# wuwuz/Pacmann

Measured on AMD Instinct MI355X. Metric: private queries/sec + PIR-scan HBM GB/s, SIFT1M d=128 at 1/2/4/8 GPUs, higher is better.
Workload: dtype u64

## Files before the change

pacmann_amd/csrc/pm_ctx.cpp:

```cpp
#include "pm_host.h"

static thread_local std::string g_err;
namespace pmh {
int fail(int code, const std::string& msg) { g_err = msg; return code; }
}

extern "C" const char* pm_last_error(void) { return g_err.c_str(); }

static constexpr AesTables kAes{};
extern "C" int pm_expand_key(const uint8_t key[16], uint32_t rk[44]) {
  uint8_t w[176];
  memcpy(w, key, 16);
  uint8_t rcon = 1;
  for (int i = 16; i < 176; i += 4) {
    uint8_t t[4] = {w[i - 4], w[i - 3], w[i - 2], w[i - 1]};
    if (i % 16 == 0) {
      uint8_t u = t[0];
      t[0] = kAes.sbox[t[1]] ^ rcon; t[1] = kAes.sbox[t[2]]; t[2] = kAes.sbox[t[3]]; t[3] = kAes.sbox[u];
      rcon = AesTables::gmul(rcon, 2);
    }
    for (int k = 0; k < 4; ++k) w[i + k] = w[i - 16 + k] ^ t[k];
  }
  memcpy(rk, w, 176);
  return 0;
// ... 25 lines not shown
  if (const char* rc = getenv("PM_ROWS_CHECK")) c->rows_check = atoi(rc);
  c->hash_mult.resize(pmk::step_max_e());
  for (size_t w = 0; w < c->hash_mult.size(); ++w) c->hash_mult[w] = row_hash_mult(w);
  if (const char* pw = getenv("PM_PUBLISH_WAIT")) c->publish_wait = pw[0] != '0';
  if (c->publish_wait) {
    for (auto& e : c->done_ring)
      if (hipEventCreateWithFlags(&e, hipEventDisableTiming | hipEventReleaseToSystem) != hipSuccess) {
        delete c;
        return fail(PM_EHIP, "hipEventCreateWithFlags(step completion) failed");
      }
    c->done_ev = c->done_ring[0];
  }
  if (const char* rs = getenv("PM_REPL_SIDE")) c->repl_side = rs[0] != '0';
  const char* ng = getenv("PM_NO_GUESS");
  c->no_guess = ng && ng[0] == '1';
  hipError_t e = hipStreamCreateWithFlags(&c->stream, hipStreamNonBlocking);
  if (e != hipSuccess) { delete c; return fail(PM_EHIP, hipGetErrorString(e)); }
  *out = c;
  return 0;
}
extern "C" void pm_ctx_destroy(pm_ctx* c) { if (c) { (void)hipSetDevice(c->device); delete c; } }
extern "C" int pm_ctx_sync(pm_ctx* c) { HIPCHK(hipStreamSynchronize(c->stream)); HIPCHK(hipGetLastError()); return 0; }
extern "C" int pm_ctx_mem_info(pm_ctx* c, uint64_t* free_b, uint64_t* total_b) {
  if (!c) return fail(PM_EINVAL, "ctx is NULL");
  HIPCHK(hipSetDevice(c->device));
  size_t f = 0, t = 0;
  HIPCHK(hipMemGetInfo(&f, &t));
  if (free_b) *free_b = f;
  if (total_b) *total_b = t;
  return 0;
}
static std::mutex g_tl_mu;
static hipEvent_t g_tl_base = nullptr;
extern "C" int pm_timing_enable(pm_ctx* c, int on) {
  c->timing = on;
  if (on >= 2) {
    std::lock_guard<std::mutex> lk(g_tl_mu);
    if (!g_tl_base) {
      HIPCHK(hipEventCreate(&g_tl_base));
      HIPCHK(hipEventRecord(g_tl_base, c->stream));
    }
  }
  return 0;
}
extern "C" int pm_timing_timeline(pm_ctx* c, const char* path) {
  if (!c || !path) return fail(PM_EINVAL, "NULL argument");
  HIPCHK(hipStreamSynchronize(c->stream));
  std::lock_guard<std::mutex> lk(g_tl_mu);
  if (!g_tl_base) return fail(PM_EINVAL, "no timeline (kernel timing level 2 never enabled)");
  FILE* f = fopen(path, "a");
  if (!f) return fail(PM_EINVAL, std::string("cannot open ") + path);
  for (auto& t : c->launches) {
    float a = 0, b = 0;
    if (hipEventElapsedTime(&a, g_tl_base, t.a) != hipSuccess || hipEventElapsedTime(&b, g_tl_base, t.b) != hipSuccess)
      continue;
    fprintf(f, "%s,%.3f,%.3f,%p\n", t.name.c_str(), a * 1e3, b * 1e3, (void*)c);
  }
  fclose(f);
  return 0;
}
namespace pmh {
std::atomic<int> g_verify_records{0};
std::atomic<int> g_device_loop{-1};
std::atomic<int> g_rccl_timeout_s{-1};
std::atomic<int> g_fault_drl_query{-1};
}
extern "C" int pm_set_option(const char* name, int value) {
  if (!name) return fail(PM_EINVAL, "NULL argument");
  if (!strcmp(name, "verify_records")) { g_verify_records.store(value < 0 ? 0 : value); return 0; }
  if (!strcmp(name, "rccl_timeout_s")) { g_rccl_timeout_s.store(value); return 0; }
  if (!strcmp(name, "device_loop")) { g_device_loop.store(value < 0 ? -1 : value); return 0; }
  if (!strcmp(name, "fault_drl_query")) { g_fault_drl_query.store(value); return 0; }
  if (!strcmp(name, "aes_bs")) { pmk::set_aes_bs(value); return 0; }
  if (!strcmp(name, "fold_rot")) {
    if (value < -1 || value > 1) return fail(PM_EINVAL, "fold_rot takes 1, 0 or -1");
    pmk::set_fold_rot(value);
    return 0;
  }
  if (!strcmp(name, "fold_pack")) {
    if (value < -1 || value > 1) return fail(PM_EINVAL, "fold_pack takes 1, 0 or -1");
    pmk::set_fold_pack(value);
    return 0;
  }
  if (pmk::set_option(name, value)) return fail(PM_EINVAL, std::string("unknown option ") + name);
  return 0;
}
extern "C" int pm_step_plan(const pm_step_shape* in, pm_step_forms* out) {
  if (!in || !out) return fail(PM_EINVAL, "NULL argument");
  if (in->kind > (uint32_t)pmk::STEP_DEVICE || in->nsub == 0 || in->np == 0) return fail(PM_EINVAL, "bad step shape");
  pmk::StepShape s{};
  s.np = in->np; s.nsub = in->nsub; s.np_live = in->np_live; s.max_per_part = in->max_per_part;
  s.maxPH = in->maxPH; s.maxSS = in->maxSS; s.E = in->E; s.ph8 = in->ph8 != 0;
  s.of_caller((int)in->kind, true);
  s.unfused = in->no_fuse != 0; s.no_split = in->no_split != 0; s.no_guess = in->no_guess != 0;
  const pmk::StepPlan p = pmk::step_plan(s, pmk::step_opts());
  static_assert(sizeof out->counter / sizeof out->counter[0] == pmk::STAGE_COUNT, "one slot per launch of a plan");
  *out = pm_step_forms{};
  for (int i = 0; i < pmk::STAGE_COUNT; ++i) {
    const pmk::StepLaunch& l = p.at[i];
    if (l.form < 0) continue;
    out->counter[i] = kHostTimerName[pm_ctx::step_counter(i, l.form)];
    out->grid_x[i] = l.gx; out->grid_y[i] = l.gy; out->block[i] = l.block;
  }
  out->nhelp = p.nhelp; out->nsplit = p.nsplit; out->qw = p.qw; out->np_live = p.np_live; out->cblk = p.cblk;
  out->no_guess = p.no_guess; out->qset = p.qset; out->args_valid = s.args_valid;
  return 0;
}
extern "C" int pm_fold_image_map(uint32_t cs, uint32_t ss, uint32_t E, uint32_t dim, int packed, uint64_t x0,
                                 uint64_t n, uint64_t* row, uint32_t* word, uint8_t* is_packed, uint64_t* nitems,
                                 uint32_t* npk_out) {
  if ((n && (!row || !word || !is_packed)) || !nitems || !npk_out) return fail(PM_EINVAL, "NULL argument");
  if ((cs != 512 && cs != 1024) || ss == 0 || ss % 4 || E < 4 || E % 2) return fail(PM_EINVAL, "not a fold image shape");
  const uint32_t npk = packed ? pmk::fold_pack_shape(E, dim) : 0;
  if (packed && (!npk || cs != 512)) return fail(PM_EINVAL, "these entries have no packed fold image");
  *nitems = pmk::fold_image_words(ss, E, cs, npk) / 2;
  *npk_out = npk;
  if (x0 > *nitems || n > *nitems - x0) return fail(PM_EINVAL, "items past the image");
  pmk::fold_image_map(cs, ss, npk, x0, n, row, word, is_packed);
  return 0;
}
extern "C" int pm_timing_reset(pm_ctx* c) {
  HIPCHK(hipStreamSynchronize(c->stream));
  for (auto& t : c->launches) { c->pool.push_back(t.a); c->pool.push_back(t.b); }
  c->launches.clear();
  for (int i = 0; i < HT_COUNT; ++i) { c->host_n[i] = 0; c->host_ms[i] = 0; }
  return 0;
}
extern "C" int pm_timing_get(pm_ctx* c, const char* name, uint64_t* launches, double* total_ms,
                             double* bytes) {
  HIPCHK(hipStreamSynchronize(c->stream));
  uint64_t n = 0; double ms = 0, by = 0;
  if (strncmp(name, "host_", 5) == 0) {
    for (int i = 0; i < HT_COUNT; ++i)
      if (strcmp(name, kHostTimerName[i]) == 0) { n = c->host_n[i]; ms = c->host_ms[i]; }
    if (launches) *launches = n;
    if (total_ms) *total_ms = ms;
    if (bytes) *bytes = 0;
    return 0;
  }
  for (auto& t : c->launches) {
    if (t.name != name) continue;
    float x = 0;
    HIPCHK(hipEventElapsedTime(&x, t.a, t.b));
    ++n; ms += x; by += t.bytes;
  }
  if (launches) *launches = n;
  if (total_ms) *total_ms = ms;
  if (bytes) *bytes = by;
  return 0;
}

#if defined(PM_STEP_STAMPS) || defined(PM_MR_STAMPS) || defined(PM_ANSWER_STAMPS)
namespace pmh {
int dump_stamps(hipStream_t st, const char* path, const void* hdr, size_t hdr_bytes, const DevBuf& buf, uint64_t count) {
  HIPCHK(hipStreamSynchronize(st));
  std::vector<uint64_t> t(count);
  HIPCHK(hipMemcpy(t.data(), buf.p, count * 8, hipMemcpyDeviceToHost));
  static std::mutex mu;
  std::lock_guard<std::mutex> lk(mu);
  if (FILE* f = fopen(path, "ab")) {
    fwrite(hdr, 1, hdr_bytes, f);
    fwrite(t.data(), 8, count, f);
    fclose(f);
  }
  return 0;
}
// ... 95 lines not shown
```

pacmann_amd/csrc/pm_devloop.cpp:

```cpp
#include "pm_engine.h"

static bool device_loop_on() {
  const int o = g_device_loop.load();
  if (o >= 0) return o != 0;
  static const int env = [] { const char* e = getenv("PM_DEVICE_LOOP"); return e ? atoi(e) : 1; }();
  return env != 0;
}
static uint32_t pow2_at_least(uint64_t x) { uint32_t c = 1; while (c < x) c *= 2; return c; }

struct DrlShape { uint32_t n = 0, qn = 0, kcap = 0, cmask = 0; };
static bool drl_plan(pm_graph** gs, uint32_t S, uint64_t q, int k, int step, int parallel, DrlShape* sh) {
  if (!device_loop_on() || S == 0 || step <= 0 || parallel <= 0 || k <= 0 || (uint32_t)parallel > pmk::kDrlMaxParallel)
    return false;
  const pm_graph* g0 = gs[0];
  const Engine& e0 = g0->pir->e;
  const uint64_t m = g0->m, n = (uint64_t)parallel * m, P = e0.P;
  if (m == 0 || m > 64 || n > pmk::kDrlMaxN || n * m > pmk::kDrlMaxNM || P == 0 || P > 64) return false;
  const uint64_t qn = n / P;
  if (qn == 0 || qn > pmk::step_max_sub_per_part() || e0.B == 0) return false;
  const uint64_t kcap = pow2_at_least((uint64_t)parallel + (uint64_t)step * n);
  if (kcap > pmk::kDrlMaxKcap || (uint64_t)k > kcap || pmk::team_round_lds(kcap, n, m) > 64 * 1024) return false;
  uint64_t maxq = ~0ull;
  for (uint32_t i = 0; i < S; ++i) {
    const pm_graph* g = gs[i];
// ... 105 lines not shown
    HIPCHK(hipMemcpy(g0->dgraph->p, g0->graph, g0->n * m * 4, hipMemcpyHostToDevice));
  }
  CHK(T.sess.reserve(S * sizeof(DrlSess)));
  CHK(T.dummy.reserve((uint64_t)S * P * 8));
  CHK(T.batch.reserve((uint64_t)S * n * 4));
  CHK(T.heap.reserve((uint64_t)S * kcap * 8));
  CHK(T.ktab.reserve((uint64_t)S * 2 * kcap * 8));
  CHK(T.knb.reserve((uint64_t)S * kcap * m * 4));
  CHK(T.kdist.reserve((uint64_t)S * kcap * 4));
  CHK(T.kid.reserve((uint64_t)S * kcap * 4));
  CHK(T.ctabp.reserve(S * 8));
  CHK(T.answers.reserve(std::max<uint64_t>(8, (uint64_t)S * q * k * 8)));
  CHK(G.buf.reserve(T.nsub, S * P, (G.maxPH + 63) / 64, pmk::step_match_blocks(G.maxPH), G.E));
  CHK(T.gid.reserve((uint64_t)T.nsub * 8));
  CHK(T.out.reserve(step_out_bytes(T.nsub, G.E)));
  CHK(T.allq.reserve(std::max<uint64_t>(4, (uint64_t)S * q * dim * 4)));
  CHK(T.part_bytes.reserve(P * 8));
  std::vector<DrlSess> hs(S);
  std::vector<uint64_t> dmy((uint64_t)S * P), ctp(S);
  for (uint32_t i = 0; i < S; ++i) {
    pm_graph* g = gs[i];
    Engine* e = &g->pir->e;
    hs[i] = DrlSess{g->rng.s, g->succ, 0, 0, 0, 0};
    for (uint32_t p = 0; p < P; ++p) dmy[(uint64_t)i * P + p] = e->parts[p].dummy_ctr;
    CHK(ensure_dev_cache(e, sh.cmask, st));
    ctp[i] = (uint64_t)(uintptr_t)e->dcache.p;
  }
  std::vector<uint32_t> sbv(S * P + 1);
  for (uint32_t j = 0; j <= S * P; ++j) sbv[j] = j * sh.qn;
  std::vector<double> pb(P);
  for (uint32_t p = 0; p < P; ++p) pb[p] = answer_bytes(e0.parts[p].d, G.E);
  HIPCHK(hipStreamSynchronize(st));
  HIPCHK(hipMemcpy(T.sess.p, hs.data(), S * sizeof(DrlSess), hipMemcpyHostToDevice));
  HIPCHK(hipMemcpy(T.dummy.p, dmy.data(), dmy.size() * 8, hipMemcpyHostToDevice));
  HIPCHK(hipMemcpy(T.ctabp.p, ctp.data(), S * 8, hipMemcpyHostToDevice));
  HIPCHK(hipMemcpy(G.buf.sb_d.p, sbv.data(), sbv.size() * 4, hipMemcpyHostToDevice));
  HIPCHK(hipMemcpy(T.part_bytes.p, pb.data(), P * 8, hipMemcpyHostToDevice));
  if (q) HIPCHK(hipMemcpy(T.allq.p, queries + (uint64_t)s0 * q * dim, (uint64_t)S * q * dim * 4, hipMemcpyHostToDevice));
  if (G.c->timing >= 2) {
    const uint64_t steps = q * (uint64_t)step;
    CHK(T.step_bytes.reserve(std::max<uint64_t>(8, steps * S * 8)));
    CHK(T.step_real.reserve(std::max<uint64_t>(4, steps * S * 4)));
    HIPCHK(hipMemsetAsync(T.step_bytes.p, 0, std::max<uint64_t>(8, steps * S * 8), st));
    HIPCHK(hipMemsetAsync(T.step_real.p, 0, std::max<uint64_t>(4, steps * S * 4), st));
  }
  HIPCHK(hipEventCreateWithFlags(&T.ev_end, hipEventDisableTiming));
  if (getenv("PM_DRL_STAMPS")) {
    CHK(T.stamps.reserve(16 * 8));
    HIPCHK(hipMemset(T.stamps.p, 0, 16 * 8));
  }
  DrlArgs& A = T.A;
  A.S = S; A.P = P; A.qn = sh.qn; A.n = n; A.m = m; A.parallel = (uint32_t)parallel; A.k = (uint32_t)k;
  A.E = G.E; A.dim = dim; A.kcap = kcap; A.cmask = sh.cmask; A.ns = G.ns; A.q = (uint32_t)q;
  A.N = g0->n; A.PS = e0.PS;
  A.vec16 = (G.E % 2 == 0 && dim % 4 == 0 && m % 4 == 0 && ((m / 4) & (m / 4 - 1)) == 0) ? 1u : 0u;
  A.hdr = T.out.as<PmOutHdr>();
  A.rows = (const uint64_t*)(T.out.as<char>() + (uint64_t)T.nsub * sizeof(PmOutHdr));
  A.subs = G.buf.subs_d.as<PmSub>(); A.gid = T.gid.as<uint64_t>();
  A.graph = g0->dgraph->as<uint32_t>();
  A.start_dist = G.start_dist.as<float>(); A.start_ids = G.start_ids.as<uint32_t>();
  A.sess = T.sess.as<DrlSess>(); A.dummy = T.dummy.as<uint64_t>(); A.batch = T.batch.as<uint32_t>();
  A.heap = T.heap.as<uint64_t>(); A.ktab = T.ktab.as<uint64_t>(); A.knb = T.knb.as<uint32_t>();
  A.kdist = T.kdist.as<float>(); A.kid = T.kid.as<uint32_t>(); A.ctab = T.ctabp.as<uint64_t*>();
  A.answers = T.answers.as<int64_t>(); A.part_bytes = T.part_bytes.as<double>();
  A.step_bytes = T.step_bytes.p ? T.step_bytes.as<double>() : nullptr;
  A.step_real = T.step_real.p ? T.step_real.as<uint32_t>() : nullptr;
  A.stamps = T.stamps.p ? T.stamps.as<uint64_t>() : nullptr;
  T.need.assign(S, 0);
  T.mt.assign(S, 0.0);
  return 0;
}

static int drl_step(DrlTeam& T, const DrlShape& sh) {
  StepGroup& G = T.G;
  pm_ctx* c = G.c;
  const Engine* e0 = G.es[0];
  c->sample_now = c->sample_ctr++ % 7 == 0;
  PmStep S{};
  S.parts = G.parts_d.as<PmPart>();
  G.buf.fill(S, (G.maxPH + 63) / 64, pmk::step_match_blocks(G.maxPH));
  S.subs_h = S.subs;
  S.sb_h = S.sb;
  S.done = G.done.as<uint32_t>();
  S.db = e0->db->as<uint64_t>();
  S.q = nullptr;
  step_out(S, T.out.p, T.nsub);
  S.E = G.E; S.dim = G.dim; S.nsub = T.nsub; S.np = T.S * G.Pl;
  S.np_live = S.np;
  S.token = next_token(G.token);
  step_read_window(S, e0->pf_off, e0->pf_len, G.E);
  S.rows_partial = 1;
  const size_t before = c->launches.size();
  double ans_bytes = 0;
  for (uint32_t li = 0; li < G.Pl; ++li) ans_bytes += answer_bytes(e0->parts[G.lp[li]].d, G.E) * sh.qn * T.S;
  CHK(group_step_launch(G, S, pmk::STEP_DEVICE, sh.qn, T.nsub, ans_bytes));
  for (size_t i = before; i < c->launches.size(); ++i)
    if (c->launches[i].name == "answer" || c->launches[i].name == "match_resolve" || c->launches[i].name == "hint_match")
      T.tl.emplace_back(i, T.seq - 1);
  c->host_add(HT_DEV_STEPS, 0.0);
  return 0;
}

static void drl_round(DrlTeam& T, uint32_t mode, uint64_t qi) {
  pm_ctx* c = T.G.c;
  DrlArgs A = T.A;
  A.mode = mode;
  A.qi = (uint32_t)qi;
  A.seq = T.seq;
  if (mode != DRL_END) T.seq++;
  c->timed_ext("team_round", 0, [&](pmk::PmEvents ev) { pmk::team_round(c->stream, A, ev); }, 2);
}

static int drl_begin(DrlTeam& T, uint64_t qi, uint64_t q) {
  StepGroup& G = T.G;
  hipStream_t st = G.c->stream;
  const uint32_t dim = G.dim;
  HIPCHK(hipMemcpy2DAsync(G.qbuf.p, (size_t)dim * 4, T.allq.as<float>() + qi * dim, (size_t)q * dim * 4,
                          (size_t)dim * 4, T.S, hipMemcpyDeviceToDevice, st));
  const uint64_t nrows = (uint64_t)T.S * G.ns;
  if (nrows)
    G.c->timed("l2_rows", (double)nrows * G.dim * 4, [&] {
      pmk::l2_rows(st, T.gs[0]->dvec->as<float>(), G.dim, nrows, G.start_ids.as<uint32_t>(), G.qbuf.as<float>(), G.dim,
                   G.start_dist.as<float>(), G.ns);
    });
  drl_round(T, DRL_BEGIN, qi);
  return 0;
}
static int drl_query_all(std::vector<std::unique_ptr<DrlTeam>>& teams, const DrlShape& sh, uint64_t qi, uint64_t q,
                         int step) {
  for (auto& t : teams) CHK(drl_begin(*t, qi, q));
  for (int r = 0; r < step; ++r)
    for (auto& t : teams) {
      CHK(drl_step(*t, sh));
      drl_round(*t, r + 1 == step ? DRL_END : DRL_MID, qi);
    }
  HIPCHK(hipGetLastError());
  for (auto& t : teams) {
    for (uint32_t i = 0; i < t->S; ++i) {
      pm_graph* g = t->gs[i];
      Engine* e = &g->pir->e;
      e->FBN += (uint64_t)step * (sh.n / e->B);
      e->QMIP += (uint64_t)step * sh.qn;
      g->total += (uint64_t)step * sh.n;
    }
    t->G.c->host_add(HT_DEV_QUERIES, (double)t->S);
  }
  return 0;
}

static int drl_team_finish(DrlTeam& T, uint64_t q, int k, int64_t* answers) {
  StepGroup& G = T.G;
  HIPCHK(hipStreamSynchronize(G.c->stream));
  const uint32_t S = T.S, P = (uint32_t)G.es[0]->P;
  if (q) HIPCHK(hipMemcpy(answers + (uint64_t)T.s0 * q * k, T.answers.p, (uint64_t)S * q * k * 8, hipMemcpyDeviceToHost));
  std::vector<DrlSess> hs(S);
  std::vector<uint64_t> dmy((uint64_t)S * P);
  HIPCHK(hipMemcpy(hs.data(), T.sess.p, S * sizeof(DrlSess), hipMemcpyDeviceToHost));
  HIPCHK(hipMemcpy(dmy.data(), T.dummy.p, dmy.size() * 8, hipMemcpyDeviceToHost));
  std::vector<uint32_t> fq(P);
  for (uint32_t i = 0; i < S; ++i) {
    pm_graph* g = T.gs[i];
    Engine* e = &g->pir->e;
    g->rng.s = hs[i].rng;
    g->succ = hs[i].succ;
    HIPCHK(hipMemcpy(fq.data(), e->fqn.p, P * 4, hipMemcpyDeviceToHost));
    for (uint32_t p = 0; p < P; ++p) {
      e->parts[p].dummy_ctr = dmy[(uint64_t)i * P + p];
// ... 150 lines not shown
```

pacmann_amd/csrc/pm_engine.cpp:

```cpp
#include "pm_engine.h"

static void derive_key(uint64_t seed, uint64_t part, uint64_t epoch, uint8_t key[16]) {
  uint64_t r1 = hash4(seed, DOM_KEY, part, epoch, 0), r2 = hash4(seed, DOM_KEY, part, epoch, 1);
  memcpy(key, &r1, 8);
  memcpy(key + 8, &r2, 8);
}

static void part_params(PartHost& ph, uint64_t N, uint64_t F) {
  uint64_t target = (uint64_t)(2 * std::sqrt((double)N));
  uint64_t cs = 1;
  while (cs < target) cs *= 2;
  uint64_t ss = (uint64_t)std::ceil((double)N / (double)cs);
  ss = (ss + 3) / 4 * 4;
  const uint64_t thr = 8;
  uint64_t maxq = (uint64_t)(std::sqrt((double)N) * std::log((double)N));
  uint64_t k = (uint64_t)std::ceil(std::log(2.0) * (double)(F + 1));
  uint64_t phn = (k * cs + thr - 1) / thr * thr;
  uint64_t qpc = 3 * (uint64_t)((double)maxq / (double)ss);
  qpc = (qpc + thr - 1) / thr * thr;
  ph.d.N = N;
  ph.d.CS = (uint32_t)cs;
  uint32_t lg = 0; while ((1ull << lg) < cs) ++lg;
  ph.d.log2CS = lg;
  ph.d.SS = (uint32_t)ss;
// ... 23 lines not shown
                         const uint64_t* rawDB, uint64_t F, uint64_t seed, bool batch,
                         uint32_t shard, uint32_t nshards, const Engine* server,
                         const DbGen* gen, uint32_t coord_words) {
  if (nshards == 0 || shard >= nshards) return fail(PM_EINVAL, "shard must be < nshards");
  if (!ctx) return fail(PM_EINVAL, "ctx is NULL");
  if (!rawDB && N && !server && !gen) return fail(PM_EINVAL, "rawDB is NULL");
  if (gen && gen->kind == 1 && (uint64_t)(gen->dim + gen->m) * 4 != Ebytes)
    return fail(PM_EINVAL, "graph entry size must be 4 * (dim + m)");
  if (server && server->ctx->device != ctx->device) return fail(PM_EINVAL, "a client shares the server DB of its own device only");
  if (N == 0) return fail(PM_EINVAL, "DBSize must be > 0");
  if (Ebytes < 8) return fail(PM_EINVAL, "DBEntryByteNum must be >= 8");
  HIPCHK(hipSetDevice(ctx->device));
  g->ctx = ctx; g->is_batch = batch;
  g->N = N; g->Ebytes = Ebytes; g->E = Ebytes / 8; g->F = F; g->seed = seed;
  if (batch) {
    g->B = B;
    g->P = B / 2;
    if (g->P == 0) return fail(PM_EINVAL, "BatchSize must be >= 2");
    g->PS = (N + g->P - 1) / g->P;
    if (g->PS > 1 && g->PS < (1ull << 32)) g->ps_magic = ~0ull / g->PS + 1;
  } else {
    g->P = 1; g->PS = N;
  }
  g->parts.resize(g->P);
  if (g->E > pmk::step_max_e()) return fail(PM_EINVAL, "DBEntrySize above the step kernel's LDS limit");
  g->shard = shard; g->nshards = nshards;
  uint64_t off_tag = 0, off_pp = 0, off_par = 0, off_ridx = 0, off_rval = 0, off_hist = 0, off_ar = 0,
           off_tab = 0, off_tabT = 0, off_cur = 0, off_db = 0;
  for (uint64_t i = 0; i < g->P; ++i) {
    PartHost& ph = g->parts[i];
    uint64_t start = i * g->PS, end = std::min((i + 1) * g->PS, N);
    if (end <= start) return fail(PM_EINVAL, "empty partition (DBSize too small for BatchSize)");
    part_params(ph, end - start, F);
    ph.owned = i % nshards == shard;
    if (!ph.owned) {
      ph.d.seed = seed; ph.d.idx = i;
      continue;
    }
    g->owned_list.push_back((uint32_t)i);
    if (ph.d.CS > 32768) return fail(PM_EINVAL, "ChunkSize > 32768 unsupported (16-bit prep offsets)");
    if (ph.d.SS > pmk::step_max_ss()) return fail(PM_EINVAL, "SetSize above the step kernel's LDS limit");
    if ((uint64_t)ph.d.H >= (1ull << 29)) return fail(PM_EINVAL, "tag space >= 2^29 (util.go:161)");
    ph.d.row0 = off_db; off_db += end - start;
    ph.d.seed = seed; ph.d.idx = i;
    g->maxH = std::max(g->maxH, ph.d.H);
    g->maxCS = std::max(g->maxCS, ph.d.CS);
    g->minCS = std::min(g->minCS, ph.d.CS);
    g->maxPH = std::max(g->maxPH, ph.d.PH);
    g->ph8 = g->ph8 && ph.d.PH % 8 == 0;
    g->maxSS = std::max(g->maxSS, ph.d.SS);
    g->maxRepl = std::max(g->maxRepl, ph.d.SS * ph.d.Qpc);
    ph.d.tag = (uint32_t*)(uintptr_t)off_tag; off_tag += ph.d.H;
    ph.d.pp = (uint32_t*)(uintptr_t)off_pp; off_pp += ph.d.PH;
    ph.d.parity = (uint64_t*)(uintptr_t)off_par; off_par += (uint64_t)ph.d.H * g->E;
    ph.d.ridx = (uint32_t*)(uintptr_t)off_ridx; off_ridx += (uint64_t)ph.d.SS * ph.d.Qpc;
    ph.d.rval = (uint64_t*)(uintptr_t)off_rval; off_rval += (uint64_t)ph.d.SS * ph.d.Qpc * g->E;
    ph.d.hist = (uint32_t*)(uintptr_t)off_hist; off_hist += ph.d.SS;
    ph.d.arena = (uint64_t*)(uintptr_t)off_ar; off_ar += (uint64_t)ph.d.MaxQ * g->E;
    ph.d.tab = (uint16_t*)(uintptr_t)off_tab; off_tab += (uint64_t)ph.d.H * ph.d.SS;
    ph.d.curk = cur_k(ph.d.PH, ph.d.SS);
    ph.d.cur = (uint16_t*)(uintptr_t)off_cur; off_cur += cur_words(ph.d.PH, ph.d.SS, ph.d.curk);
    ph.d.tabT = (uint16_t*)(uintptr_t)off_tabT; off_tabT += tabT_words(ph.d.H, ph.d.SS);
    ph.cache.reserve(ph.d.MaxQ);
  }
  CHK(g->zero16.reserve(64));
  HIPCHK(hipMemset(g->zero16.p, 0, 64));
  if (server) g->db = server->db;
  else CHK(g->db->reserve(std::max<uint64_t>(8, off_db * g->E * 8)));
  for (uint32_t i : server ? std::vector<uint32_t>{} : g->owned_list) {
    const uint64_t start = (uint64_t)i * g->PS, rows = g->parts[i].d.N;
    uint64_t* dst = g->db->as<uint64_t>() + g->parts[i].d.row0 * g->E;
    if (gen && gen->kind == 0)
      pmk::db_synth(ctx->stream, dst, start, rows, (uint32_t)g->E, gen->seed);
    else if (gen)
      pmk::graph_synth(ctx->stream, dst, start, rows, N, gen->dim, gen->m, gen->seed);
    else
      HIPCHK(hipMemcpy(dst, rawDB + start * g->E, rows * g->E * 8, hipMemcpyHostToDevice));
  }
  if (gen) {
    HIPCHK(hipGetLastError());
    HIPCHK(hipStreamSynchronize(ctx->stream));
  }
  uint64_t off_img = 0;
  if (!g->owned_list.empty() && pmk::fold_image_ok(g->minCS, g->maxCS, (uint32_t)g->E)) {
    if (server) {
      g->img_npk = server->img_npk;
    } else if (const uint32_t npk = pmk::fold_pack_slices(g->minCS, g->maxCS, (uint32_t)g->E, coord_words)) {
      DevBuf flag;
      CHK(flag.reserve(64));
      if (pmk::coord_low_zero(ctx->stream, g->db->as<uint64_t>(), off_db, (uint32_t)g->E, coord_words, flag.as<uint32_t>()))
        g->img_npk = npk;
      HIPCHK(hipGetLastError());
    }
    for (uint32_t i : g->owned_list) {
      PmPart& d = g->parts[i].d;
      d.img = (const uint64_t*)(uintptr_t)off_img;
      off_img += pmk::fold_image_words(d.SS, (uint32_t)g->E, (uint32_t)g->maxCS, g->img_npk);
    }
    size_t free_b = 0, total_b = 0;
    if (!server && hipMemGetInfo(&free_b, &total_b) == hipSuccess && off_img * 8 > free_b / 4) {
      for (uint32_t i : g->owned_list) g->parts[i].d.img = nullptr;
      off_img = 0;
    } else if (server && !server->img->p) {
      for (uint32_t i : g->owned_list) g->parts[i].d.img = nullptr;
      off_img = 0;
    }
    if (!off_img) g->img_npk = 0;
  }
  if (off_img) {
    if (server) {
      g->img = server->img;
    } else {
      CHK(g->img->reserve(off_img * 8));
      for (uint32_t i : g->owned_list) {
        const PmPart& d = g->parts[i].d;
        pmk::fold_image(ctx->stream, g->img->as<uint64_t>() + (uintptr_t)d.img, g->db->as<uint64_t>() + d.row0 * g->E,
                        d.N, d.SS, (uint32_t)g->E, (uint32_t)g->maxCS, g->img_npk);
      }
      HIPCHK(hipGetLastError());
      HIPCHK(hipStreamSynchronize(ctx->stream));
    }
  }
  CHK(g->tag.reserve(off_tag * 4));
  CHK(g->pp.reserve(off_pp * 4));
  CHK(g->parity.reserve(off_par * 8));
  CHK(g->ridx.reserve(off_ridx * 4));
  CHK(g->rval.reserve(off_rval * 8));
  CHK(g->hist.reserve(off_hist * 4));
  CHK(g->fqn.reserve(g->P * 4));
  CHK(g->arena.reserve(std::max<uint64_t>(8, off_ar * 8)));
  const bool need_tab = pmk::fold_needs_tab(g->minCS, g->maxCS, (uint32_t)g->E, off_img != 0);
  if (need_tab) CHK(g->tab.reserve(off_tab * 2));
  CHK(g->tabT.reserve(off_tabT * 2));
  CHK(g->cur.reserve(std::max<uint64_t>(2, off_cur * 2)));
  CHK(g->done.reserve(4 * (3 + 16 * 4096)));
  {
    const uint32_t init[3] = {1u << 31, 0, 0};
    HIPCHK(hipMemcpy(g->done.p, init, sizeof init, hipMemcpyHostToDevice));
  }
  {
    g->gran_words = (g->maxPH + 63) / 64;
    const size_t n = (size_t)kArgSubs * (8 + 64 + 2 * g->gran_words + 8) * 8;
    CHK(g->gran.reserve(n));
    HIPCHK(hipMemset(g->gran.p, 0, n));
    CHK(g->err_h.reserve(64));
    memset(g->err_h.p, 0, 64);
  }
  CHK(g->parts_d.reserve(g->P * sizeof(PmPart)));
  CHK(g->owned_d.reserve(std::max<size_t>(1, g->owned_list.size()) * sizeof(PmPart)));
  CHK(g->parts_stage.reserve((g->P + g->owned_list.size()) * sizeof(PmPart)));
  for (uint64_t i = 0; i < g->P; ++i) {
    PmPart& d = g->parts[i].d;
    if (!g->parts[i].owned) continue;
    d.tag = g->tag.as<uint32_t>() + (uintptr_t)d.tag;
    d.pp = g->pp.as<uint32_t>() + (uintptr_t)d.pp;
    d.parity = g->parity.as<uint64_t>() + (uintptr_t)d.parity;
    d.ridx = g->ridx.as<uint32_t>() + (uintptr_t)d.ridx;
    d.rval = g->rval.as<uint64_t>() + (uintptr_t)d.rval;
    d.hist = g->hist.as<uint32_t>() + (uintptr_t)d.hist;
    d.fqn = g->fqn.as<uint32_t>() + i;
    d.arena = g->arena.as<uint64_t>() + (uintptr_t)d.arena;
    d.tabT = g->tabT.as<uint16_t>() + (uintptr_t)d.tabT;
    d.tab = need_tab ? g->tab.as<uint16_t>() + (uintptr_t)d.tab : nullptr;
    d.cur = g->cur.as<uint16_t>() + (uintptr_t)d.cur;
    d.img = off_img ? g->img->as<uint64_t>() + (uintptr_t)d.img : nullptr;
  }
  HIPCHK(hipMemsetAsync(g->fqn.p, 0, g->P * 4, ctx->stream));
  HIPCHK(hipMemsetAsync(g->hist.p, 0, off_hist * 4, ctx->stream));
  HIPCHK(hipStreamSynchronize(ctx->stream));
  return 0;
}
}

static int upload_parts(Engine* g) {
  std::vector<PmPart> v(g->P), w;
  for (uint64_t i = 0; i < g->P; ++i) v[i] = g->parts[i].d;
  for (uint32_t i : g->owned_list) w.push_back(g->parts[i].d);
  HIPCHK(hipMemcpyAsync(g->parts_d.p, v.data(), g->P * sizeof(PmPart), hipMemcpyHostToDevice,
                        g->ctx->stream));
  if (!w.empty())
    HIPCHK(hipMemcpyAsync(g->owned_d.p, w.data(), w.size() * sizeof(PmPart), hipMemcpyHostToDevice,
                          g->ctx->stream));
  HIPCHK(hipStreamSynchronize(g->ctx->stream));
  return 0;
}

static int upload_parts_async(Engine* g, hipStream_t st) {
  if (g->ctx->stream != st && hipStreamQuery(g->ctx->stream) != hipSuccess) {
    if (!g->order_ev) HIPCHK(hipEventCreateWithFlags(&g->order_ev, hipEventDisableTiming));
    HIPCHK(hipEventRecord(g->order_ev, g->ctx->stream));
    HIPCHK(hipStreamWaitEvent(st, g->order_ev, 0));
  }
  const size_t no = g->owned_list.size();
  if (g->stage_ev) HIPCHK(hipEventSynchronize(g->stage_ev));
  else HIPCHK(hipEventCreateWithFlags(&g->stage_ev, hipEventDisableTiming));
  CHK(g->parts_stage.reserve((g->P + no) * sizeof(PmPart)));
  PmPart* h = g->parts_stage.as<PmPart>();
  for (uint64_t i = 0; i < g->P; ++i) h[i] = g->parts[i].d;
  for (size_t i = 0; i < no; ++i) h[g->P + i] = g->parts[g->owned_list[i]].d;
  HIPCHK(hipMemcpyAsync(g->parts_d.p, h, g->P * sizeof(PmPart), hipMemcpyHostToDevice, st));
  if (no) HIPCHK(hipMemcpyAsync(g->owned_d.p, h + g->P, no * sizeof(PmPart), hipMemcpyHostToDevice, st));
  HIPCHK(hipEventRecord(g->stage_ev, st));
  return 0;
// ... 291 lines not shown
                  (unsigned long)row[0], (unsigned long)(it == ph.shadow.end() ? 0 : it->second[0]), (unsigned long)dev[0]);
        }
      }
    }
  }
  for (uint32_t s = 0; s < nsub; ++s) {
    const PmOutHdr& h = g->hdr[s];
    if (h.status == ST_OK) {
      PartHost& ph = g->parts[g->subs[s].part];
      ph.fqn++;
      ph.cache.put(g->subs[s].idx, h.ref);
    } else if (h.status == ST_DUP) {
      const uint32_t r = h.ref - base;
      memcpy(g->rows + (uint64_t)s * E, g->rows + (uint64_t)r * E, E * 8);
      g->hdr[s].dist = g->hdr[r].dist;
    }
  }
#ifdef PM_STAMPS
  {
    std::vector<uint64_t> t(64);
    (void)hipMemcpy(t.data(), g->buf.stamps.p, 64 * 8, hipMemcpyDeviceToHost);
    g->stamp_sum.resize(64, 0.0);
    for (int i = 1; i < 64; ++i)
    {
      const uint64_t base = i >= 48 ? t[48] : i >= 41 ? t[41] : t[0];
      if (t[i] && base && i != 41 && i != 48) g->stamp_sum[i] += (double)(t[i] - base);
    }
    g->stamp_n++;
  }
#endif
}

#if defined(PM_STEP_STAMPS) || defined(PM_MR_STAMPS) || defined(PM_ANSWER_STAMPS)
struct LaunchStamps {
  const char* file = nullptr;
  uint64_t words = 0;
  int begin(const char* f, std::atomic<int>* first, hipStream_t st, StepBufs& B, PmStep& S, uint64_t n) {
    if (!f || (first && first->fetch_add(1) >= 40)) return 0;
    CHK(B.stamps.reserve(n * 8));
    HIPCHK(hipMemsetAsync(B.stamps.p, 0, n * 8, st));
    S.stamps = B.stamps.as<uint64_t>();
    file = f; words = n;
    return 0;
  }
  int end(hipStream_t st, const StepBufs& B, PmStep& S, const void* hdr, size_t hdr_bytes) {
    if (!file) return 0;
    S.stamps = nullptr;
    return dump_stamps(st, file, hdr, hdr_bytes, B.stamps, words);
  }
};
#endif

int step_chain(pm_ctx* c, StepBufs& B, PmStep& S, const pmk::StepShape& shape, uint32_t nreal, double ans_bytes,
               const std::function<int()>& after_resolve) {
  hipStream_t st = c->stream;
  if (shape.desc_shared != (S.subs == S.subs_h && S.sb == S.sb_h))
    return fail(PM_EINVAL, "step_chain: the descriptor is not where the step's shape says");
  const pmk::StepPlan plan = pmk::step_plan(shape, pmk::step_opts());
  S.args_valid = shape.args_valid ? 1u : 0u;
  S.nsplit = plan.nsplit; S.qw = plan.qw; S.np_live = plan.np_live; S.cblk = plan.cblk; S.nhelp = plan.nhelp; S.no_guess = plan.no_guess;
  const uint32_t nsub = S.nsub;
  if (plan.qset) {
    CHK(B.qset.reserve((uint64_t)nsub * plan.qw * 2));
    S.qset = B.qset.as<uint16_t>();
  }
  if (plan.nsplit > 1) {
    CHK(B.part_x.reserve((uint64_t)nsub * plan.nsplit * (S.E & ~3u) * 8));
    S.part_x = B.part_x.as<uint64_t>();
  }
  const bool fused = plan.at[pmk::STAGE_FUSED].form >= 0;
  if (fused) {
    if (plan.nhelp && !B.helpg.p) {
      const size_t nh = (size_t)kArgSubs * kStepHelpMax * kHelpGran * 8;
      CHK(B.helpg.reserve(nh));
      HIPCHK(hipMemsetAsync(B.helpg.p, 0, nh, st));
    }
    S.helpg = B.helpg.as<uint64_t>();
  }
  auto run = [&](int stage, const char* name, double bytes) {
    const int form = plan.at[stage].form;
    if (form < 0) return;
    c->timed_ext(name, bytes, [&](pmk::PmEvents ev) { pmk::step_launch(st, S, plan, stage, ev); }, 2);
    c->host_add(pm_ctx::step_counter(stage, form), stage == pmk::STAGE_FUSED ? plan.nhelp : 0.0);
  };
#ifdef PM_STEP_STAMPS
  LaunchStamps ss;
  const uint32_t sh[4] = {plan.at[pmk::STAGE_FUSED].gx, nsub, pmk::step_match_blocks(shape.maxPH), S.np};
  if (fused) CHK(ss.begin(getenv("PM_STAMP_FILE"), nullptr, st, B, S, (uint64_t)sh[0] * 8));
#endif
  run(pmk::STAGE_FUSED, "step", ans_bytes);
#ifdef PM_STEP_STAMPS
  CHK(ss.end(st, B, S, sh, sizeof sh));
#endif
#ifdef PM_MR_STAMPS
  LaunchStamps ms;
  static std::atomic<int> mr_steps{0};
  const uint64_t mh = S.np;
  if (plan.at[pmk::STAGE_MR].form >= 0) CHK(ms.begin(getenv("PM_MR_STAMPS"), &mr_steps, st, B, S, mh * 8));
#endif
  run(pmk::STAGE_MR, "match_resolve", (double)nreal * shape.maxPH);
#ifdef PM_MR_STAMPS
  CHK(ms.end(st, B, S, &mh, sizeof mh));
#endif
  run(pmk::STAGE_MATCH, "hint_match", (double)nreal * shape.maxPH);
  run(pmk::STAGE_RESOLVE, "resolve", 0);
  if (after_resolve) CHK(after_resolve());
  run(pmk::STAGE_GATHER, "gather", ans_bytes);
#ifdef PM_ANSWER_STAMPS
  LaunchStamps as;
  static std::atomic<int> ans_steps{0};
  const uint64_t ah = nsub;
  if (!fused) CHK(as.begin(getenv("PM_ANSWER_STAMPS"), &ans_steps, st, B, S, ah * 8));
#endif
  run(pmk::STAGE_ANSWER, "answer", plan.nsplit > 1 ? 0 : ans_bytes);
#ifdef PM_ANSWER_STAMPS
  CHK(as.end(st, B, S, &ah, sizeof ah));
#endif
  return 0;
}

int engine_step(Engine* g, const float* q_dev, uint32_t dim) {
  auto t_begin = Clock::now();
  pm_ctx* c = g->ctx;
  hipStream_t st = c->stream;
  const uint32_t nsub = (uint32_t)g->subs.size();
  if (nsub == 0) return 0;
  const uint64_t E = g->E;
  const uint32_t words = (g->maxPH + 63) / 64, cblk = pmk::step_match_blocks(g->maxPH);
  StepBufs& B = g->buf;
  CHK(B.reserve(nsub, (uint32_t)g->P, words, cblk, E));
  const size_t dsub = nsub * sizeof(PmSub);
  CHK(B.desc_h.reserve(dsub + (g->P + 1) * 4));
  CHK(B.out_h.reserve(step_out_bytes(nsub, E)));
  char* dh = B.desc_h.as<char>();
  memcpy(dh, g->subs.data(), dsub);
  memcpy(dh + dsub, g->sb.data(), (g->P + 1) * 4);
  PmStep S{};
  S.parts = g->parts_d.as<PmPart>();
  S.subs_h = (const PmSub*)dh;
  S.sb_h = (const uint32_t*)(dh + dsub);
  B.fill(S, words, cblk);
  if (words <= g->gran_words) {
    uint64_t* gb = g->gran.as<uint64_t>();
    S.recg = gb;
    S.specg = gb + kArgSubs * 8;
    S.bitsg = gb + kArgSubs * (8 + 64);
    S.resg = gb + kArgSubs * (8 + 64 + 2 * (uint64_t)g->gran_words);
    S.err_h = g->err_h.as<uint32_t>();
  }
  S.done = g->done.as<uint32_t>();
#ifdef PM_STAMPS
  CHK(B.stamps.reserve(g->P * 64 * 8));
  HIPCHK(hipMemsetAsync(B.stamps.p, 0, g->P * 64 * 8, st));
  S.stamps = B.stamps.as<uint64_t>();
#endif
  S.db = g->db->as<uint64_t>();
  S.q = q_dev;
  step_out(S, B.out_h.p, nsub);
  S.E = (uint32_t)E; S.dim = q_dev ? dim : 0; S.nsub = nsub; S.np = (uint32_t)g->P;
  S.token = next_token(g->step_token);
  step_read_window(S, g->pf_off, g->pf_len, E);
  S.rows_partial = host_rows_partial(c, g->rows_partial);
  uint32_t nreal = 0;
  for (auto& x : g->subs) nreal += x.kind == SUB_REAL;
  pmk::StepShape shape{};
  shape.np = (uint32_t)g->P; shape.nsub = nsub; shape.maxPH = g->maxPH; shape.maxSS = g->maxSS; shape.E = (uint32_t)E; shape.ph8 = g->ph8;
  for (uint64_t p = 0; p < g->P; ++p) {
    const uint32_t n = g->sb[p + 1] - g->sb[p];
    shape.max_per_part = std::max(shape.max_per_part, n);
    shape.np_live += n > 0;
  }
  shape.of_caller(pmk::STEP_ENGINE, S.recg && S.err_h);
  shape.unfused = c->no_fuse || c->debug_sync; shape.no_split = c->no_split; shape.no_guess = c->no_guess;
  if (shape.args_valid) {
    memcpy(S.subs_a, g->subs.data(), dsub);
    memcpy(S.sb_a, g->sb.data(), (g->P + 1) * 4);
  }
  double ans_bytes = 0;
  for (auto& x : g->subs)
    if (x.kind == SUB_REAL || x.kind == SUB_DUMMY) ans_bytes += answer_bytes(g->parts[x.part].d, E);
  std::function<int()> dump_res;
  if (c->debug_sync) dump_res = [&]() -> int {
    std::vector<PmRes> rr(nsub);
    HIPCHK(hipMemcpy(rr.data(), S.res, nsub * sizeof(PmRes), hipMemcpyDeviceToHost));
    for (uint32_t s = 0; s < nsub; ++s) {
      const PmPart& d = g->parts[g->subs[s].part].d;
      const PmRes& r = rr[s];
      const bool bad = (r.status == ST_OK && (r.hit >= d.PH || r.slot >= d.MaxQ || r.chunk >= d.SS || r.ing >= d.Qpc)) ||
                       (r.status == ST_CACHED && r.slot >= d.MaxQ) || (r.status == ST_DUP && r.slot >= nsub) ||
                       (r.status > ST_SKIP) || (r.status > ST_ERANGE && r.status < ST_DUMMY);
      fprintf(stderr, "[pm] res s=%u part=%u kind=%u idx=%lu -> st=%u hit=%u chunk=%u ing=%u tag=%u pp=%u slot=%u flags=%u%s\n",
              s, g->subs[s].part, g->subs[s].kind, (unsigned long)g->subs[s].idx, r.status, r.hit, r.chunk, r.ing,
              r.tag, r.pp, r.slot, r.flags, bad ? "  <-- BAD" : "");
    }
    return 0;
  };
  CHK(step_chain(c, B, S, shape, nreal, ans_bytes, dump_res));
  g->step_seq = c->record_done(st);
  HIPCHK(hipGetLastError());
  c->host_add(HT_STEP_LAUNCH, ms_since(t_begin));
  CHK(wait_and_post(g, S, nsub, t_begin));
  if (S.err_h && *(volatile uint32_t*)S.err_h) {
    *(volatile uint32_t*)S.err_h = 0;
    return fail(PM_EHIP, "k_step: a hand-off wait timed out (results of this step are invalid)");
  }
  return 0;
}
}

static void add_sub(Engine* g, uint32_t p, bool real, uint64_t local, uint64_t gid) {
  PartHost& ph = g->parts[p];
  if (!ph.owned) return;
  PmSub s{p, SUB_NONE, 0};
  if (!real) {
    s.kind = SUB_DUMMY; s.idx = ph.dummy_ctr++;
  } else {
    s.kind = SUB_REAL; s.idx = local;
    if (const uint32_t* slot = ph.cache.find(local)) { s.kind = SUB_HOSTCACHE; s.idx = *slot; }
  }
  g->subs.push_back(s);
  g->sub_gid.push_back(gid);
}
static void begin_step(Engine* g) {
  g->subs.clear(); g->sub_gid.clear();
  g->sb.assign(g->P + 1, 0);
}
static void close_partition(Engine* g, uint32_t p) {
  for (uint64_t i = p + 1; i <= g->P; ++i) g->sb[i] = (uint32_t)g->subs.size();
}

namespace pmh {
void print_stamps(const Engine& e) {
#ifdef PM_STAMPS
  if (!e.stamp_n) return;
  fprintf(stderr, "[pm-stamps] mean shader clocks since kernel start over %lu steps (1-40 k_resolve part 0, 42-47 k_match, 49-63 k_answer):", (unsigned long)e.stamp_n);
  for (size_t i = 1; i < e.stamp_sum.size(); ++i)
    if (e.stamp_sum[i] > 0) fprintf(stderr, " %zu:%.0f", i, e.stamp_sum[i] / e.stamp_n);
  fprintf(stderr, "\n");
#else
// ... 411 lines not shown
```

pacmann_amd/csrc/pm_engine.h:

```cpp
#pragma once
#include "pm_host.h"

#include <functional>

struct DbGen;
struct Engine;
struct pm_graph;
struct StepGroup;
struct StepBufs;
struct ShardComb;

namespace pmh {
int engine_create(pm_ctx* ctx, Engine* g, uint64_t N, uint64_t Ebytes, uint64_t B,
                  const uint64_t* rawDB, uint64_t F, uint64_t seed, bool batch,
                  uint32_t shard = 0, uint32_t nshards = 1, const Engine* server = nullptr,
                  const DbGen* gen = nullptr, uint32_t coord_words = 0);
int ensure_host_cache(Engine* g);
int engine_prep_host(Engine* g, uint64_t p0, uint64_t p1, std::vector<uint64_t>& todo,
                     hipStream_t st = nullptr);
int engine_prep_launch(pm_ctx* c, const Engine* g, const PmPart* dp, int np, const PmPart* host_parts,
                       uint32_t clients = 1, bool sync = true);
int wait_done(pm_ctx* sc, uint64_t seq);
int poll_done(pm_ctx* sc, uint64_t seq, bool* ready);
int wait_step(pm_ctx* c, const PmOutHdr* hdr, uint32_t nsub, uint32_t token, const char* rows,
// ... 74 lines not shown
  bool emplace(uint64_t k, uint32_t v) {
    if (find(k)) return false;
    put(k, v);
    return true;
  }
  template <class F> void for_each(F&& f) const {
    for (const Slot& x : slot) if (x.gen == cur) f(x.key, x.val);
  }
};

struct StepBufs {
  DevBuf subs_d, sb_d, bits, cand, meta, spec, res_d, ans, part_x, stamps;
  DevBuf qset;
  DevBuf helpg;
  HostBuf desc_h, out_h;
  int reserve(uint32_t nsub, uint32_t np, uint32_t words, uint32_t cblk, uint64_t E) {
    CHK(subs_d.reserve(nsub * sizeof(PmSub)));
    CHK(sb_d.reserve((np + 1) * 4));
    CHK(bits.reserve((uint64_t)nsub * words * 8));
    CHK(cand.reserve((uint64_t)nsub * cblk * 6 * 4));
    CHK(meta.reserve((uint64_t)nsub * 2 * 4));
    CHK(spec.reserve((uint64_t)nsub * 64 * 4));
    CHK(res_d.reserve(nsub * sizeof(PmRes)));
    CHK(ans.reserve((uint64_t)nsub * E * 8));
    return 0;
  }
  void fill(PmStep& S, uint32_t words, uint32_t cblk) const {
    S.subs = subs_d.as<PmSub>();
    S.sb = sb_d.as<uint32_t>();
    S.bits = bits.as<uint64_t>();
    S.cand = cand.as<uint32_t>();
    S.meta = meta.as<uint32_t>();
    S.spec = spec.as<uint32_t>();
    S.res = res_d.as<PmRes>();
    S.ans = ans.as<uint64_t>();
    S.words = words;
    S.cblk = cblk;
  }
};
static inline size_t step_out_bytes(uint32_t nsub, uint64_t E) { return nsub * sizeof(PmOutHdr) + (size_t)nsub * E * 8; }
static inline void step_out(PmStep& S, void* out, uint32_t nsub) {
  S.hdr_h = (PmOutHdr*)out;
  S.rows_h = (uint64_t*)((char*)out + nsub * sizeof(PmOutHdr));
}
static inline uint32_t next_token(uint32_t& token) {
  if (++token == 0) ++token;
  return token;
}
static inline void step_read_window(PmStep& S, size_t pf_off, size_t pf_len, uint64_t E) {
  const size_t off = std::min<size_t>(pf_off, E * 8);
  const size_t end = std::min<size_t>(E * 8, off + std::min<size_t>(pf_len, E * 8));
  S.pf_w0 = (uint32_t)(off / 8);
  S.pf_w1 = (uint32_t)((end + 7) / 8);
}
static inline uint32_t host_rows_partial(const pm_ctx* c, bool partial) {
  return partial && !c->verify_rows && !c->debug_cache ? 1u : 0u;
}
struct PartHost {
  PmPart d{};
  bool owned = true;
  uint64_t epoch_ctr = 0, fqn = 0, dummy_ctr = 0;
  uint64_t maxq64 = 0;
  FlatMap cache;
  std::unordered_map<uint64_t, std::vector<uint64_t>> shadow;
};

struct Engine {
  pm_ctx* ctx = nullptr;
  bool is_batch = false;
  uint64_t N = 0, E = 0, Ebytes = 0, F = 0, seed = 0;
  uint64_t B = 0, P = 1, PS = 0;
  uint64_t ps_magic = 0;
  uint64_t part_of(uint64_t id) const {
    return ps_magic && id < (1ull << 32) ? (uint64_t)(((unsigned __int128)id * ps_magic) >> 64) : id / PS;
  }
  uint32_t shard = 0, nshards = 1;
  bool skipPrep = false;
  uint64_t FBN = 0, QMIP = 0, Support = 0, prepCount = 0;
  double prepTime = 0, storage = 0, commOn = 0, commOff = 0;

  std::shared_ptr<DevBuf> db = std::make_shared<DevBuf>();
  std::shared_ptr<DevBuf> img = std::make_shared<DevBuf>();
  uint32_t img_npk = 0;
  DevBuf zero16, parts_d, owned_d, tag, pp, parity, ridx, rval, hist, fqn, arena, tab, tabT, cur, done, gran;
  HostBuf parts_stage;
  hipEvent_t stage_ev = nullptr;
  hipEvent_t order_ev = nullptr;
  uint32_t gran_words = 0;
  std::vector<uint32_t> owned_list;
  DevBuf qoffs, ans_srv;
  StepBufs buf;
  std::vector<double> stamp_sum;
  uint64_t stamp_n = 0;
  uint32_t step_token = 0;
  uint64_t step_seq = 0;
  size_t pf_off = 0, pf_len = ~size_t(0);
  bool rows_partial = false;
  HostBuf err_h, src_h;
  HostBuf stage_h;
  hipEvent_t dev_ev = nullptr;
  ~Engine() {
    if (dev_ev) (void)hipEventDestroy(dev_ev);
    if (stage_ev) (void)hipEventDestroy(stage_ev);
    if (order_ev) (void)hipEventDestroy(order_ev);
  }
  std::vector<PartHost> parts;
  uint32_t maxH = 0, maxPH = 0, maxSS = 0, maxRepl = 0, maxCS = 0, minCS = ~0u;
  bool ph8 = true;

  std::vector<PmSub> subs;
  std::vector<uint32_t> sb;
  std::vector<uint64_t> sub_gid;
  PmOutHdr* hdr = nullptr;
  uint64_t* rows = nullptr;
  std::vector<std::vector<uint64_t>> pq;
  FlatMap resp_map;
  std::vector<uint64_t> resp_rows;
  std::vector<float> resp_dist;
  std::vector<uint8_t> resp_ok;
  std::vector<char> slow;
  uint64_t qn = 0;
  uint64_t prep_gen = 0;
  std::vector<uint64_t> zero_row;
  DevBuf dcache;
  uint32_t dcache_cmask = 0;
  bool cache_on_dev = false, dcache_valid = false;
};

static inline double answer_bytes(const PmPart& d, uint64_t E) {
  const double rows = std::min((double)d.SS, (double)d.N / (double)d.CS);
  return rows * (double)E * 8 + 4.0 * d.SS + 8.0 * E;
}

struct DbGen { int kind; uint64_t seed; uint32_t dim, m; };

struct pm_batchpir { Engine e; ~pm_batchpir() { print_stamps(e); } };

struct SplitMix {
  uint64_t s;
  uint64_t next() { s += 0x9e3779b97f4a7c15ULL; uint64_t z = s;
    z = (z ^ (z >> 30)) * 0xbf58476d1ce4e5b9ULL; z = (z ^ (z >> 27)) * 0x94d049bb133111ebULL;
    return z ^ (z >> 31); }
  uint64_t intn(uint64_t n) { return next() % n; }
};
struct VD { float dist; int64_t id; };

struct pm_graph {
  pm_ctx* ctx = nullptr;
  uint64_t n = 0, dim = 0, m = 0;
  bool nonprivate = false, skipPrep = false;
  uint64_t pir_seed = 0;
  SplitMix rng{0};
  std::shared_ptr<const std::vector<float>> vec_own;
  std::shared_ptr<const std::vector<uint32_t>> graph_own;
  const float* vectors = nullptr;
  const uint32_t* graph = nullptr;
  std::shared_ptr<DevBuf> dvec = std::make_shared<DevBuf>();
  std::shared_ptr<DevBuf> dgraph = std::make_shared<DevBuf>();
  uint32_t shard = 0, nshards = 1;
  bool synth = false;
  uint64_t data_seed = 0;
  DevBuf dstartvec;
  std::vector<uint8_t> okv;
  const uint32_t* true_nb(uint64_t id, uint32_t* tmp) const {
    if (!synth) return graph + id * m;
    const uint64_t kg = sm64(data_seed + DOM_SYNTH_NB);
// ... 94 lines not shown
```

pacmann_amd/csrc/pm_group.cpp:

```cpp
#include "pm_engine.h"

struct SpinBarrier {
  std::atomic<uint32_t> count{0}, gen{0};
  uint32_t n = 1;
  void wait() {
    const uint32_t g0 = gen.load(std::memory_order_acquire);
    if (count.fetch_add(1, std::memory_order_acq_rel) + 1 == n) {
      count.store(0, std::memory_order_relaxed);
      gen.fetch_add(1, std::memory_order_release);
    } else {
      while (gen.load(std::memory_order_acquire) == g0) std::this_thread::yield();
    }
  }
};

struct ShardComb {
  pm_combine_fn fn = nullptr;
  void* user = nullptr;
  bool model_peers = false;
  uint32_t NG = 1;
  uint64_t* const* bufs = nullptr;
  std::atomic<uint64_t> ticket{0};
  std::atomic<bool> abort{false};
};
// ... 100 lines not shown
    if (!ss.ok || ss.step != G.nstep) staged = false;
    nsub += ss.n;
  }
  if (staged && pmk::step_args_fit(nsub, np)) staged = false;
  G.nstep++;
  PmSub* const stage = G.stage_h.as<PmSub>();
  if (staged) {
    uint32_t off = 0;
    for (uint32_t s = 0; s < G.S; ++s) {
      const StepGroup::SessStage& ss = G.stg[s];
      G.base[s] = off;
      const uint32_t n = in[s] ? ss.n : 0;
      if (n && off != s * G.stride) memmove(stage + off, stage + (uint64_t)s * G.stride, (size_t)n * sizeof(PmSub));
      for (uint32_t li = 0; li < G.Pl; ++li) G.sb.push_back(G.sb.back() + (in[s] ? ss.pc[li] : 0));
      if (in[s]) {
        max_per_part = std::max(max_per_part, ss.maxpp);
        np_live += ss.live;
        ans_bytes += ss.bytes;
        nreal += ss.nreal;
      }
      off += n;
    }
  } else {
    G.subs.clear();
    for (uint32_t s = 0; s < G.S; ++s) {
      Engine* e = G.es[s];
      G.base[s] = (uint32_t)G.subs.size();
      for (uint32_t li = 0; li < G.Pl; ++li) {
        const uint32_t p = G.lp[li];
        if (in[s]) {
          for (uint32_t j = e->sb[p]; j < e->sb[p + 1]; ++j) {
            PmSub x = e->subs[j];
            x.part = s * G.Pl + li;
            G.subs.push_back(x);
            if (x.kind == SUB_REAL || x.kind == SUB_DUMMY) ans_bytes += answer_bytes(e->parts[p].d, G.E);
            nreal += x.kind == SUB_REAL;
          }
          const uint32_t n = e->sb[p + 1] - e->sb[p];
          max_per_part = std::max(max_per_part, n);
          np_live += n > 0;
        }
        G.sb.push_back((uint32_t)G.subs.size());
      }
      need = std::max(need, in[s] ? (uint32_t)G.subs.size() - G.base[s] : 0u);
    }
    nsub = (uint32_t)G.subs.size();
  }
  G.nsub = nsub;
  if (G.stage_on && need > G.stride) {
    G.stride = (need + 7) & ~7u;
    CHK(G.stage_h.reserve((size_t)G.S * G.stride * sizeof(PmSub) + (size_t)(np + 1) * 4));
    if (G.stg.size() != G.S) G.stg.resize(G.S);
  }
  if (nsub == 0) return 0;
  const uint32_t words = (G.maxPH + 63) / 64, cblk = pmk::step_match_blocks(G.maxPH);
  StepBufs& B = G.buf;
  CHK(B.reserve(nsub, np, words, cblk, G.E));
  const size_t dsub = nsub * sizeof(PmSub);
  char* dh;
  if (staged) {
    dh = G.stage_h.as<char>();
    memcpy(dh + dsub, G.sb.data(), (np + 1) * 4);
  } else {
    CHK(B.desc_h.reserve(dsub + (np + 1) * 4));
    dh = B.desc_h.as<char>();
    memcpy(dh, G.subs.data(), dsub);
    memcpy(dh + dsub, G.sb.data(), (np + 1) * 4);
  }
  PmStep S{};
  S.parts = G.parts_d.as<PmPart>();
  S.subs_h = (const PmSub*)dh;
  S.sb_h = (const uint32_t*)(dh + dsub);
  B.fill(S, words, cblk);
  if (!pmk::step_args_fit(nsub, np)) {
    CHK(G.desc_d.reserve(dsub + (np + 1) * 4));
    HIPCHK(hipMemcpyAsync(G.desc_d.p, dh, dsub + (np + 1) * 4, hipMemcpyHostToDevice, st));
    S.subs_h = G.desc_d.as<PmSub>();
    S.sb_h = (const uint32_t*)(G.desc_d.as<char>() + dsub);
    S.subs = const_cast<PmSub*>(S.subs_h);
    S.sb = const_cast<uint32_t*>(S.sb_h);
  }
  S.done = G.done.as<uint32_t>();
  Engine* e0 = G.es[0];
  S.db = e0->db->as<uint64_t>();
  S.q = nullptr;
  if (G.comb) {
    CHK(G.out_d.reserve(step_out_bytes(nsub, G.E)));
    step_out(S, G.out_d.p, nsub);
  } else {
    CHK(B.out_h.reserve(step_out_bytes(nsub, G.E)));
    step_out(S, B.out_h.p, nsub);
  }
  S.E = G.E; S.dim = G.dim; S.nsub = nsub; S.np = np;
  S.np_live = np_live;
  if (pmk::step_args_fit(nsub, np)) {
    memcpy(S.subs_a, G.subs.data(), dsub);
    memcpy(S.sb_a, G.sb.data(), (np + 1) * 4);
  }
  S.token = next_token(G.token);
  step_read_window(S, e0->pf_off, e0->pf_len, G.E);
  S.rows_partial = host_rows_partial(c, G.rows_partial);
  return group_step_launch(G, S, pmk::STEP_SHARED, max_per_part, nreal, ans_bytes);
}

static void prefetch_session(StepGroup& G, uint32_t s, const pm_graph* g) {
  const Engine* e = G.es[s];
  const uint32_t n = (uint32_t)e->subs.size();
  const PmOutHdr* hdr = G.buf.out_h.as<PmOutHdr>() + G.base[s];
  const char* rows = G.buf.out_h.as<char>() + (size_t)G.nsub * sizeof(PmOutHdr) + (size_t)G.base[s] * G.E * 8;
  for (uint32_t j = 0; j < n; j += 2) __builtin_prefetch(hdr + j);
  for (uint32_t j = 0; j < n; ++j)
    for (uint32_t w = G.pf_w0; w < G.pf_w1; w += 8) __builtin_prefetch(rows + ((size_t)j * G.E + w) * 8);
  if (g->graph)
    for (size_t b = 0; b < g->batch.size(); ++b) __builtin_prefetch(&g->graph[(uint64_t)g->batch[b] * g->m]);
}

static int group_collect(StepGroup& G, uint32_t s) {
  Engine* e = G.es[s];
  const uint32_t n = (uint32_t)e->subs.size();
  for (uint32_t j = 0; j < n; ++j)
    if (e->subs[j].kind == SUB_REAL) e->parts[e->subs[j].part].cache.prefetch(e->subs[j].idx);
  PmOutHdr* hdr = G.buf.out_h.as<PmOutHdr>();
  uint64_t* rows = (uint64_t*)(G.buf.out_h.as<char>() + (size_t)G.nsub * sizeof(PmOutHdr));
  auto t_wait = Clock::now();
  CHK(wait_step(e->ctx, hdr + G.base[s], n, G.token, (const char*)(rows + (uint64_t)G.base[s] * G.E),
                (size_t)G.E * 8, (size_t)G.pf_w0 * 8, (size_t)(G.pf_w1 - G.pf_w0) * 8, G.seq, G.c));
  e->ctx->host_add(HT_STEP_WAIT, ms_since(t_wait));
  auto tp = Clock::now();
  post_results(e, hdr, rows, n, G.base[s], G.token);
  e->ctx->host_add(HT_STEP_POST, ms_since(tp));
  return 0;
}

static int group_start_dist(StepGroup& G, pm_graph** gs) {
  hipStream_t st = G.c->stream;
  float* qst = G.qstage.as<float>();
  HIPCHK(hipMemcpyAsync(G.qbuf.p, qst, (uint64_t)G.S * G.dim * 4, hipMemcpyHostToDevice, st));
  const uint64_t nrows = (uint64_t)G.S * G.ns;
  if (nrows) {
    const bool ids = gs[0]->dvec->p != nullptr;
    G.c->timed("l2_rows", (double)nrows * G.dim * 4, [&] {
      pmk::l2_rows(st, ids ? gs[0]->dvec->as<float>() : G.start_vec.as<float>(), G.dim, nrows,
                   ids ? G.start_ids.as<uint32_t>() : nullptr, G.qbuf.as<float>(), G.dim, G.start_dist.as<float>(),
                   G.ns);
    });
    HIPCHK(hipMemcpyAsync(qst + (uint64_t)G.S * G.dim, G.start_dist.p, nrows * 4, hipMemcpyDeviceToHost, st));
  }
  HIPCHK(hipStreamSynchronize(st));
  return 0;
}

namespace pmh {
int prep_clients(pm_ctx* c, DevBuf& pbuf, const std::vector<uint32_t>& lp, const std::vector<Engine*>& who,
                        const std::vector<double*>* mt, HostBuf* stage, hipEvent_t* stage_ev) {
  if (who.empty()) return 0;
  for (Engine* e : who)
    if ((e->img->p != nullptr) != (who[0]->img->p != nullptr))
      return fail(PM_EINVAL, "grouped clients were created with and without the fold image");
  auto t0 = Clock::now();
  std::vector<PmPart> hp;
  std::vector<uint64_t> todo;
  for (Engine* e : who) {
    e->FBN = 0; e->QMIP = 0;
    CHK(engine_prep_host(e, 0, e->P, todo, c->stream));
  }
  for (uint32_t p : lp)
    for (Engine* e : who) hp.push_back(e->parts[p].d);
// ... 898 lines not shown
```

pacmann_amd/csrc/pm_host.h:

```cpp
#define PM_HOST_TU 1
#pragma once
#include "pm_internal.h"
#include "pm_aes.h"
#include "../../include/pacmann.h"

#include <dlfcn.h>
#include <hip/hip_runtime.h>
#include <rccl/rccl.h>

#include <algorithm>
#include <atomic>
#include <cstdio>
#include <cstdlib>
#include <chrono>
#include <condition_variable>
#include <cmath>
#include <cstring>
#include <memory>
#include <string>
#include <mutex>
#include <thread>
#include <unordered_map>
#include <vector>

using namespace pm;

struct DevBuf;

namespace pmh {
int fail(int code, const std::string& msg);
extern std::atomic<int> g_verify_records;
extern std::atomic<int> g_device_loop;
extern std::atomic<int> g_rccl_timeout_s;
extern std::atomic<int> g_fault_drl_query;
int dump_stamps(hipStream_t st, const char* path, const void* hdr, size_t hdr_bytes, const DevBuf& buf, uint64_t count);
}
using namespace pmh;

#define HIPCHK(x)                                                                         \
  do {                                                                                    \
    hipError_t e_ = (x);                                                                  \
    if (e_ != hipSuccess)                                                                 \
      return fail(PM_EHIP, std::string(#x) + ": " + hipGetErrorString(e_));               \
  } while (0)
#define CHK(x)            \
  do {                    \
    int r_ = (x);         \
    if (r_ != 0) return r_; \
  } while (0)

struct DevBuf {
  void* p = nullptr;
  size_t n = 0;
  ~DevBuf() { if (p) (void)hipFree(p); }
  int reserve(size_t bytes) {
    if (bytes <= n) return 0;
    if (p) { (void)hipFree(p); p = nullptr; n = 0; }
    if (bytes == 0) return 0;
    hipError_t e = hipMalloc(&p, bytes);
    if (e != hipSuccess) return fail(PM_ENOMEM, "hipMalloc(" + std::to_string(bytes) + "): " + hipGetErrorString(e));
    n = bytes;
    return 0;
  }
  template <class T> T* as() const { return (T*)p; }
};
struct HostBuf {
  void* p = nullptr;
  size_t n = 0;
  ~HostBuf() { if (p) (void)hipHostFree(p); }
  int reserve(size_t bytes) {
    if (bytes <= n) return 0;
    if (p) { (void)hipHostFree(p); p = nullptr; n = 0; }
    hipError_t e = hipHostMalloc(&p, bytes, hipHostMallocCoherent | hipHostMallocMapped);
    if (e != hipSuccess) return fail(PM_ENOMEM, std::string("hipHostMalloc: ") + hipGetErrorString(e));
    memset(p, 0, bytes);
    n = bytes;
    return 0;
  }
  template <class T> T* as() const { return (T*)p; }
};

enum HostTimer : int { HT_STEP_LAUNCH, HT_STEP_WAIT, HT_STEP_POST, HT_BATCH_QUERY, HT_GVI_PARSE, HT_SEARCH_KNN, HT_KNN_INIT, HT_KNN_BATCH, HT_KNN_UPDATE, HT_KNN_FINAL, HT_WAIT_FIRST, HT_WAIT_ALL, HT_ROWS_SEEN, HT_ROWS_TORN, HT_WAIT_DONE, HT_COMBINE, HT_COMBINE_TURN, HT_PATH_MATCH, HT_PATH_MATCH_PART, HT_PATH_MATCH_PART8, HT_PREP_SETS, HT_REC_VERIFIED, HT_REC_BAD, HT_REC_DROPPED, HT_REC_FAILED, HT_REC_PEER, HT_REC_UNEXPLAINED, HT_FOLD_ROT512, HT_FOLD_ROT1024, HT_FOLD_OTHER, HT_FOLD_PIPE, HT_FOLD_BLK, HT_FOLD_GATHER, HT_FOLD_ROT512P, HT_DEV_STEPS, HT_DEV_QUERIES, HT_KNN_BATCH_FALLBACK, HT_PATH_STEP, HT_PATH_RESOLVE_LDS, HT_PATH_RESOLVE_G, HT_PATH_MR_S2, HT_PATH_MR_S4, HT_PATH_MR_GENERAL, HT_PATH_GATHER, HT_PATH_ANSWER_P5, HT_PATH_ANSWER_P, HT_PATH_ANSWER_S, HT_PATH_ANSWER_G, HT_COUNT };
static const char* const kHostTimerName[HT_COUNT] = {"host_step_launch", "host_step_wait", "host_step_post", "host_batch_query", "host_gvi_parse", "host_search_knn", "host_knn_init", "host_knn_batch", "host_knn_update", "host_knn_final", "host_wait_first_token", "host_wait_all_tokens", "host_rows_seen", "host_rows_torn", "host_wait_done", "host_combine", "host_combine_turn", "host_path_match", "host_path_match_part", "host_path_match_part8", "host_prep_sets", "host_records_verified", "host_records_bad", "host_records_dropped", "host_records_failed", "host_records_peer", "host_records_unexplained", "host_fold_rot512", "host_fold_rot1024", "host_fold_other", "host_fold_pipe", "host_fold_blk", "host_fold_gather", "host_fold_rot512p", "host_dev_steps", "host_dev_queries", "host_knn_batch_fallback", "host_path_step", "host_path_resolve_lds", "host_path_resolve_g", "host_path_mr_s2", "host_path_mr_s4", "host_path_mr_general", "host_path_gather", "host_path_answer_p5", "host_path_answer_p", "host_path_answer_s", "host_path_answer_g"};
static_assert(HT_PATH_ANSWER_G - HT_PATH_STEP + 1 == pmk::FORM_COUNT, "one counter per step form, in the order of pmk::FORM_*");

struct TimedLaunch { std::string name; hipEvent_t a, b; double bytes; };

struct pm_ctx {
  int device = 0;
  hipStream_t stream = nullptr;
  int timing = 0;
  bool sample_now = true;
  uint64_t sample_ctr = 0;
  bool no_fuse = false;
  bool no_split = false;
  bool no_guess = false;
  bool verify_rows = false;
  bool debug_cache = false;
  bool log_steps = false;
  bool debug_sync = false;
  bool repl_side = true;
  hipStream_t side = nullptr;
  hipEvent_t side_ev[2] = {};
  std::mutex side_mu;
  int rows_check = 2;
  std::vector<uint64_t> hash_mult;
  bool publish_wait = true;
  static constexpr uint32_t kDoneRing = 64;
  hipEvent_t done_ev = nullptr;
  hipEvent_t done_ring[kDoneRing] = {};
  std::atomic<uint64_t> done_rec{0}, done_seen{0};
  std::mutex done_mu, rec_mu;
  uint64_t record_done(hipStream_t st) {
    if (!publish_wait) return 0;
    std::lock_guard<std::mutex> lk(rec_mu);
    const uint64_t seq = done_rec.load(std::memory_order_relaxed) + 1;
    (void)hipEventRecord(done_ring[seq % kDoneRing], st);
    done_rec.store(seq, std::memory_order_release);
    return seq;
  }
  std::string last_kernel;
  uint64_t host_n[HT_COUNT] = {};
  double host_ms[HT_COUNT] = {};
  void host_add(HostTimer t, double ms) { host_n[t]++; host_ms[t] += ms; }
  static HostTimer step_counter(int stage, int form) {
    if (stage != pmk::STAGE_MATCH) return (HostTimer)(HT_PATH_STEP + form);
    return form == pmk::MATCH_PART8 ? HT_PATH_MATCH_PART8 : form == pmk::MATCH_PART ? HT_PATH_MATCH_PART : HT_PATH_MATCH;
  }
  std::vector<TimedLaunch> launches;
  std::vector<hipEvent_t> pool;
  hipEvent_t ev() {
    if (!pool.empty()) { hipEvent_t e = pool.back(); pool.pop_back(); return e; }
    hipEvent_t e; (void)hipEventCreate(&e); return e;
  }
  template <class F> void timed(const char* name, double bytes, F&& f, int level = 1) {
    last_kernel = name;
    if (debug_sync) {
      f();
      hipError_t e = hipStreamSynchronize(stream);
      if (e != hipSuccess) fprintf(stderr, "[pm] kernel %s failed: %s\n", name, hipGetErrorString(e));
      return;
    }
    if (timing < level) { f(); return; }
    TimedLaunch t{name, ev(), ev(), bytes};
    (void)hipEventRecord(t.a, stream);
    f();
    (void)hipEventRecord(t.b, stream);
    launches.push_back(t);
  }
  template <class F> void timed_ext(const char* name, double bytes, F&& f, int level) {
    last_kernel = name;
    if (debug_sync) { timed(name, bytes, [&] { f(pmk::PmEvents{}); }, level); return; }
    if (timing < level || (timing == 3 && level == 2 && !sample_now)) { f(pmk::PmEvents{}); return; }
    TimedLaunch t{name, ev(), ev(), bytes};
    f(pmk::PmEvents{t.a, t.b});
    launches.push_back(t);
  }
  ~pm_ctx() {
    for (auto& t : launches) { (void)hipEventDestroy(t.a); (void)hipEventDestroy(t.b); }
    for (auto e : pool) (void)hipEventDestroy(e);
    for (auto e : done_ring) if (e) (void)hipEventDestroy(e);
    for (auto e : side_ev) if (e) (void)hipEventDestroy(e);
    if (side) (void)hipStreamDestroy(side);
    if (stream) (void)hipStreamDestroy(stream);
  }
};
// ... 5 lines not shown
```

pacmann_amd/csrc/pm_internal.h:

```cpp
#pragma once
#include <hip/hip_runtime.h>
#include <stdint.h>

#include <string>

#if defined(__HIP_DEVICE_COMPILE__) && !defined(PM_HOST_TU)
#define PM_G __attribute__((address_space(1)))
#else
#define PM_G
#endif

namespace pm {

constexpr uint32_t kDefaultProgramPoint = 0x7fffffffu;
constexpr uint64_t kDefaultValue = 0xdeadbeefULL;
constexpr uint16_t kSkip = 0xffffu;
constexpr int kBlock = 256;

enum : uint64_t { DOM_KEY = 1, DOM_REPL = 2, DOM_DUMMY = 3, DOM_SYNTH_DB = 9, DOM_SYNTH_VEC = 10, DOM_SYNTH_NB = 11 };
__host__ __device__ inline uint64_t sm64(uint64_t x) {
  uint64_t z = x + 0x9e3779b97f4a7c15ULL;
  z = (z ^ (z >> 30)) * 0xbf58476d1ce4e5b9ULL;
  z = (z ^ (z >> 27)) * 0x94d049bb133111ebULL;
  return z ^ (z >> 31);
// ... 27 lines not shown
  uint64_t seed;
  uint64_t epoch;
  uint64_t idx;
  uint32_t CS, log2CS, SS, PH, Qpc, H, MaxQ, curk;
  uint32_t rk[44];
  PM_G uint32_t* tag;
  PM_G uint32_t* pp;
  PM_G uint64_t* parity;
  PM_G uint32_t* ridx;
  PM_G uint64_t* rval;
  PM_G uint32_t* hist;
  PM_G uint32_t* fqn;
  PM_G uint64_t* arena;
  PM_G uint16_t* tab;
  PM_G uint16_t* tabT;
  PM_G uint16_t* cur;
  const PM_G float* qv;
  const PM_G uint64_t* img;
};

__host__ __device__ inline uint64_t tabT_index(uint32_t H, uint32_t t, uint32_t c) {
  return ((uint64_t)(c >> 3) * H + t) * 8 + (c & 7);
}
struct FoldImageSrc { uint64_t row; uint32_t word; bool packed; };
__host__ __device__ inline uint64_t tabT_words(uint32_t H, uint32_t SS) { return (uint64_t)((SS + 7) / 8) * 8 * H; }

#ifndef PM_CUR_K
#define PM_CUR_K 0
#endif
__host__ __device__ inline uint32_t cur_k(uint32_t PH, uint32_t SS) {
  return PM_CUR_K ? PM_CUR_K : ((uint64_t)PH * 2 > (uint64_t)SS * 128 ? 1u : 2u);
}
__host__ __device__ inline uint32_t cur_blocks(uint32_t PH) { return (PH + 7) >> 3; }
__host__ __device__ inline uint64_t cur_index(uint32_t PH, uint32_t K, uint32_t c, uint32_t h) {
  return K == 2 ? (((uint64_t)(c >> 1) * cur_blocks(PH) + (h >> 3)) * 2 + (c & 1)) * 8 + (h & 7)
                : (((uint64_t)(c / K) * cur_blocks(PH) + (h >> 3)) * K + (c % K)) * 8 + (h & 7);
}
__host__ __device__ inline uint64_t cur_row(uint32_t PH, uint32_t K, uint32_t c) { return cur_index(PH, K, c, 0); }
__host__ __device__ inline uint32_t cur_row_off(uint32_t K, uint32_t h) { return (h >> 3) * 8 * K + (h & 7); }
__host__ __device__ inline uint64_t cur_words(uint32_t PH, uint32_t SS, uint32_t K) {
  return (uint64_t)((SS + K - 1) / K) * cur_blocks(PH) * 8 * K;
}

enum : uint32_t { SUB_NONE = 0, SUB_REAL = 1, SUB_DUMMY = 2, SUB_HOSTCACHE = 3 };
enum : uint32_t {
  ST_OK = 0, ST_EBUDGET = 1, ST_ECHUNK = 2, ST_ENOHIT = 3, ST_ERANGE = 4,
  ST_DUMMY = 8, ST_CACHED = 9, ST_DUP = 10, ST_SKIP = 11
};
struct PmSub {
  uint32_t part, kind;
  uint64_t idx;
};
struct PmRes {
  uint32_t status, hit, chunk, ing;
  uint32_t tag, pp;
  uint32_t slot;
  uint32_t flags;
};
constexpr uint64_t kCsumMix = 0x9E3779B97F4A7C15ull;
__host__ __device__ inline uint64_t row_hash_mult(uint64_t w) { return sm64(w ^ 0x5851F42D4C957F2Dull) | 1ull; }
struct alignas(16) PmOutHdr {
  uint32_t status, ref;
  float dist;
  uint32_t token;
  uint64_t csum, pad;
};
#ifndef PM_KARG_SUBS
#define PM_KARG_SUBS 112
#endif
constexpr uint32_t kArgSubs = PM_KARG_SUBS, kArgParts = PM_KARG_SUBS > 1 ? 32 : 1;
constexpr uint32_t kStepHelpMax = 3, kHelpWords = 256, kHelpGran = 2 * kHelpWords + 8;
struct PmStep {
  const PM_G PmPart* parts;
  const PM_G PmSub* subs_h;
  const PM_G uint32_t* sb_h;
  PM_G PmSub* subs;
  PM_G uint32_t* sb;
  PM_G uint64_t* bits;
  PM_G uint32_t* cand;
  PM_G PmRes* res;
  PM_G uint64_t* ans;
  PM_G uint32_t* done;
  const PM_G uint64_t* db;
  const PM_G float* q;
  PM_G PmOutHdr* hdr_h;
  PM_G uint64_t* rows_h;
  PM_G uint64_t* stamps;
  PM_G uint32_t* meta;
  PM_G uint32_t* spec;
  PM_G uint64_t* recg;
  PM_G uint64_t* specg;
  PM_G uint64_t* bitsg;
  PM_G uint64_t* resg;
  PM_G uint64_t* helpg;
  uint32_t nhelp;
  PM_G uint32_t* err_h;
  uint32_t words, E, dim, nsub, np, cblk;
  uint32_t np_live;
  uint32_t pf_w0, pf_w1;
  uint32_t rows_partial;
  uint32_t no_guess;
  uint32_t nsplit;
  PM_G uint64_t* part_x;
  PM_G uint16_t* qset;
  uint32_t qw;
  uint32_t args_valid;
  uint32_t token;
  uint32_t sb_a[kArgParts + 1];
  PmSub subs_a[kArgSubs];
};

__host__ __device__ inline uint32_t drl_hash(uint32_t k) {
  uint64_t x = k;
  x ^= x >> 33; x *= 0xff51afd7ed558ccdULL; x ^= x >> 33;
  return (uint32_t)x;
}
struct DrlSess {
  uint64_t rng;
  uint64_t succ;
  uint32_t nknown, nheap;
  uint32_t pad0, pad1;
};
enum : uint32_t { DRL_BEGIN = 0, DRL_MID = 1, DRL_END = 2 };
struct DrlArgs {
  uint32_t S, P, qn, n, m, parallel, k, E, dim, kcap, cmask, ns, mode, q, qi, seq;
  uint32_t vec16;
  uint64_t N, PS;
  const PmOutHdr* hdr;
  const uint64_t* rows;
  PmSub* subs;
  uint64_t* gid;
  const uint32_t* graph;
  const float* start_dist;
  const uint32_t* start_ids;
  DrlSess* sess;
  uint64_t* dummy;
  uint32_t* batch;
  uint64_t* heap;
  uint64_t* ktab;
  uint32_t* knb;
  float* kdist;
  uint32_t* kid;
  uint64_t* const* ctab;
  int64_t* answers;
  const double* part_bytes;
  double* step_bytes;
  uint32_t* step_real;
  uint64_t* stamps;
};

struct KnbArgs {
  const float* vec;
  const uint32_t* graph;
  const uint32_t* start;
  const float* queries;
  uint32_t nq, ns, dim, m, k, max_step, parallel, kcap;
  int64_t* ids;
  int64_t* steps;
  uint32_t* needs_host;
};

}

namespace pmk {
using namespace pm;
void prep_init(hipStream_t st, const PmPart* dparts, int nparts, uint32_t maxH, uint32_t maxRepl,
               uint32_t E, bool zero_state);
void prep_offsets(hipStream_t st, const PmPart* dparts, int nparts, uint32_t maxH, uint32_t maxSS);
void set_aes_bs(int v);
enum : int { FOLD_GATHER = 0, FOLD_ROT512 = 1, FOLD_ROT1024 = 2, FOLD_PIPE = 3, FOLD_BLK = 4, FOLD_ROT512P = 5 };
int fold_form(uint32_t minCS, uint32_t maxCS, uint32_t E, bool have_img, uint32_t npk = 0);
void set_fold_rot(int v);
int prep_fold(hipStream_t st, const PmPart* dparts, int nparts, uint32_t maxH, const uint64_t* db,
              uint32_t E, uint32_t minCS, uint32_t maxCS, const uint64_t* zero16, uint32_t clients = 1,
              bool have_img = false, uint32_t minH = 0, uint32_t npk = 0);
void prep_repl(hipStream_t st, const PmPart* dparts, int nparts, uint32_t maxRepl,
               const uint64_t* db, uint32_t E);
bool fold_image_ok(uint32_t minCS, uint32_t maxCS, uint32_t E);
bool fold_needs_tab(uint32_t minCS, uint32_t maxCS, uint32_t E, bool have_img);
uint64_t fold_image_words(uint32_t SS, uint32_t E, uint32_t CS, uint32_t npk = 0);
void fold_image(hipStream_t st, uint64_t* img, const uint64_t* part_rows, uint64_t N, uint32_t SS, uint32_t E,
                uint32_t CS, uint32_t npk = 0);
void set_fold_pack(int v);
uint32_t fold_pack_shape(uint32_t E, uint32_t dim);
uint32_t fold_pack_slices(uint32_t minCS, uint32_t maxCS, uint32_t E, uint32_t dim);
bool coord_low_zero(hipStream_t st, const uint64_t* rows, uint64_t nrows, uint32_t E, uint32_t dim, uint32_t* flag);
void fold_image_map(uint32_t CS, uint32_t SS, uint32_t npk, uint64_t x0, uint64_t n, uint64_t* row, uint32_t* word,
                    uint8_t* packed);
struct PmEvents { hipEvent_t a = nullptr, b = nullptr; };
int set_option(const char* name, int value);
struct StepOpts { int match_part, match_part8, match_resolve, answer_waves, answer_nt, answer_pair, gather_split, step_help; };
StepOpts step_opts();
uint32_t step_match_blocks(uint32_t maxPH);
enum : int { STEP_ENGINE = 0, STEP_SHARED = 1, STEP_DEVICE = 2 };
inline bool step_args_fit(uint32_t nsub, uint32_t np) { return nsub <= kArgSubs && np <= kArgParts; }
struct StepShape {
  uint32_t np, nsub, np_live, max_per_part, maxPH, maxSS, E;
  bool ph8;
  bool args_valid;
  bool desc_shared;
  bool granules;
  bool unfused;
  bool no_split, no_guess;
  void of_caller(int kind, bool have_granules) {
    args_valid = kind != STEP_DEVICE && step_args_fit(nsub, np);
    desc_shared = kind == STEP_DEVICE || (kind == STEP_SHARED && !args_valid);
    granules = kind == STEP_ENGINE && have_granules;
  }
};
enum : int { MATCH_SUB = 0, MATCH_PART = 1, MATCH_PART8 = 2 };
enum : int { FORM_STEP = 0, FORM_RESOLVE_LDS, FORM_RESOLVE_G, FORM_MR_S2, FORM_MR_S4, FORM_MR_GENERAL,
             FORM_GATHER, FORM_ANSWER_P5, FORM_ANSWER_P, FORM_ANSWER_S, FORM_ANSWER_G, FORM_COUNT };
enum : int { STAGE_FUSED = 0, STAGE_MR, STAGE_MATCH, STAGE_RESOLVE, STAGE_GATHER, STAGE_ANSWER, STAGE_COUNT };
struct StepLaunch { int form = -1; uint32_t gx = 0, gy = 1, block = 0; };
struct StepPlan {
  StepLaunch at[STAGE_COUNT];
  uint32_t nhelp, nsplit, qw, np_live, cblk, no_guess;
  bool qset;
};
StepPlan step_plan(const StepShape& s, const StepOpts& O);
void step_launch(hipStream_t st, const PmStep& S, const StepPlan& plan, int stage, PmEvents ev = {});
uint32_t step_max_sub_per_part();
uint32_t step_max_ss();
uint32_t step_max_e();
void server_answer(hipStream_t st, const PmPart* dpart, const uint32_t* offs, uint32_t nq,
                   uint32_t SS, const uint64_t* db, uint32_t E, uint64_t* out);
void l2_rows(hipStream_t st, const float* rows, uint64_t row_stride_floats, uint64_t nrows,
             const uint32_t* row_ids, const float* q, uint32_t dim, float* out, uint64_t seglen = 0);
void ip_rows(hipStream_t st, const uint32_t* rows, uint64_t nrows, const uint32_t* q, uint32_t dim,
             uint32_t* per_row, uint32_t* sum);
void ip_fill(hipStream_t st, uint32_t* rows, uint64_t N, uint32_t D, uint64_t r0 = 0);
void db_synth(hipStream_t st, uint64_t* dst, uint64_t r0, uint64_t rows, uint32_t E, uint64_t db_seed);
void gather_rows(hipStream_t st, const uint64_t* const* src, uint64_t n, uint32_t E, uint64_t* out);
void graph_synth(hipStream_t st, uint64_t* dst, uint64_t r0, uint64_t rows, uint64_t n, uint32_t dim, uint32_t m,
                 uint64_t seed);
void graph_synth_vecs(hipStream_t st, const uint64_t* ids, uint64_t nids, uint32_t dim, uint64_t seed, float* out);
void pack_records(hipStream_t st, const int32_t* map, uint32_t nrec, const PmOutHdr* hdr, const uint64_t* rows,
                  uint32_t E, uint32_t w0, uint32_t W, uint64_t* rec, uint32_t nsub, uint32_t* st2, uint64_t errw);
void synth_records(hipStream_t st, const int32_t* map, const uint64_t* ids, uint32_t nrec, uint32_t npos,
                   const float* qbuf, uint32_t dim, uint32_t m, uint64_t n, uint64_t seed, uint32_t w0, uint32_t W,
                   uint64_t* rec);
void prf_batch(hipStream_t st, const uint32_t* rk, const uint64_t* tags, const uint64_t* xs,
               uint64_t n, uint64_t* out);
void team_round(hipStream_t st, const DrlArgs& A, PmEvents ev = {});
uint32_t team_round_lds(uint32_t kcap, uint32_t n, uint32_t m);
constexpr uint32_t kDrlMaxKcap = 4096, kDrlMaxN = 256, kDrlMaxNM = 8192, kDrlMaxParallel = 8;
constexpr uint32_t kKnbMaxBatch = 256, kKnbMaxM = 64, kKnbMaxLds = 160 * 1024 - 512;
uint32_t knn_batch_kcap(uint64_t parallel, uint64_t max_step, uint64_t m);
uint64_t knn_batch_lds(uint32_t kcap, uint32_t dim, uint32_t nb, uint32_t ns);
bool knn_batch_ok(uint64_t dim, uint64_t m, uint64_t ns, uint64_t max_step, uint64_t parallel);
void knn_batch(hipStream_t st, const KnbArgs& A);
uint32_t knn_pad_dim(uint32_t dim);
uint32_t knn_top();
uint32_t prune_max_list();
uint32_t prune_max_dim();
uint32_t prune_max_m();
void to_bf16(hipStream_t st, const float* rows, uint64_t n, uint32_t dim, uint32_t dp, void* out, float* norms);
void knn_prefilter(hipStream_t st, const void* X, const float* xn, uint64_t N, const void* Q, const float* qn,
                   uint64_t M, uint32_t dp, uint32_t* out, uint32_t* out_hi = nullptr);
void knn_rerank(hipStream_t st, const float* X, uint64_t N, uint32_t dim, const float* Q, uint64_t M,
                const uint32_t* cand, uint32_t K, bool self_base, uint32_t* out, float* dist, uint32_t* len);
void to_bf16x2(hipStream_t st, const float* rows, uint64_t n, uint32_t dim, uint32_t dp, void* hi, void* lo,
               float* norms, uint32_t* maxnorm);
void knn_prefilter_x3(hipStream_t st, const void* Xh, const void* Xl, const float* xn, uint64_t N, const void* Qh,
                      const void* Ql, const float* qn, uint64_t M, uint32_t dp, uint32_t* out, float* tau,
                      uint32_t* out_hi = nullptr);
float knn_cert_rel(uint32_t dp);
void knn_rerank_cert(hipStream_t st, const float* X, uint64_t N, uint32_t dim, const float* Q, uint64_t M,
                     const uint32_t* cand, uint32_t K, bool self_base, uint32_t* out, float* dist, uint32_t* len,
                     const float* qn, const float* tau, const uint32_t* maxnorm, uint32_t dp, uint64_t* list,
                     uint64_t* nlist, float* eps_out = nullptr);
void knn_brute(hipStream_t st, const float* X, uint64_t N, uint32_t dim, const float* Q, const uint64_t* list,
               uint64_t nlist, uint32_t K, bool self_base, uint32_t* out, float* dist, uint32_t* len);
void prune(hipStream_t st, const float* X, uint32_t dim, const uint32_t* verts, uint64_t nverts,
           const uint64_t* offs, uint64_t stride, const uint32_t* lens, const uint32_t* ids, uint32_t m,
           float alpha, uint32_t* out, uint32_t* out_len, uint32_t* err, const uint32_t* sorted_pos = nullptr,
           const float* dist_g = nullptr);
void cand_dist(hipStream_t st, const float* X, uint32_t dim, const uint32_t* verts, uint64_t nverts,
               const uint64_t* offs, const uint32_t* lens, const uint32_t* ids, float* dist_g);
uint32_t knn_pad_dim_wide(uint32_t dim);
void knn_prefilter_x3_w(hipStream_t st, const void* Xh, const void* Xl, const float* xn, uint64_t N, const void* Qh,
                        const void* Ql, const float* qn, uint64_t M, uint32_t dp, uint32_t* out, float* tau,
                        uint32_t* out_hi = nullptr);
void knn_brute_w(hipStream_t st, const float* X, uint64_t N, uint32_t dim, const float* Q, const uint64_t* list,
                 uint64_t nlist, uint32_t K, bool self_base, uint32_t* out, float* dist, uint32_t* len);
void prune_w(hipStream_t st, const float* X, uint32_t dim, const uint32_t* verts, uint64_t nverts,
             const uint64_t* offs, uint64_t stride, const uint32_t* lens, const uint32_t* ids, uint32_t m,
             float alpha, uint32_t* out, uint32_t* out_len, uint32_t* err, const uint32_t* sorted_pos = nullptr,
             const float* dist_g = nullptr);
}
```

pacmann_amd/csrc/pm_kernels.hip:

```cpp
#include <atomic>
#include "pm_aes.h"
#include "pm_aes_bs.h"
#include "pm_internal.h"

namespace pm {
#ifndef PM_PREP_NT
#define PM_PREP_NT 0
#endif


__device__ __forceinline__ uint32_t xor3(uint32_t a, uint32_t b, uint32_t c) {
  return __builtin_amdgcn_bitop3_b32(a, b, c, 0x96);
}
__device__ __forceinline__ uint4 xor4(uint4 a, uint4 b) {
  return make_uint4(a.x ^ b.x, a.y ^ b.y, a.z ^ b.z, a.w ^ b.w);
}

#ifndef PM_OFFS_CHUNKS
#define PM_OFFS_CHUNKS 8
#endif
constexpr int kOffsChunksPerBlock = PM_OFFS_CHUNKS;
constexpr int kOffsBlock = 1024;

#ifndef PM_OFFS_TILES
// ... 524 lines not shown
        uint32_t v[2][8];
#pragma unroll
        for (uint32_t pp = 0; pp < 2; ++pp) {
          const uint32_t ph = p0 + pp;
          uint32_t o;
          if constexpr (NCH == 4) o = __builtin_amdgcn_perm(tv[k].y, tv[k].x, psel[ph]);
          else o = __builtin_amdgcn_perm(0u, tv[k], psel[ph]);
          o = min(o, (uint32_t)CS);
          const uint32_t a = o * (LINE * 4) + cso[ph];
          const uint4 x0 = *reinterpret_cast<const uint4*>(lds0 + a);
          const uint4 x1 = *reinterpret_cast<const uint4*>(lds0 + (a ^ 16u));
          v[pp][0] = x0.x; v[pp][1] = x0.y; v[pp][2] = x0.z; v[pp][3] = x0.w;
          v[pp][4] = x1.x; v[pp][5] = x1.y; v[pp][6] = x1.z; v[pp][7] = x1.w;
        }
#pragma unroll
        for (int t = 0; t < 8; ++t)
          acc[k][t] = xor3(acc[k][t], v[0][t], v[1][t]);
      }
    }
    asm volatile("s_waitcnt vmcnt(0)" ::: "memory");
    __syncthreads();
#pragma unroll
    for (int k = 0; k < HPL; ++k) tv[k] = tn[k];
    skip_idle(tv);
  }
#pragma unroll
  for (int k = 0; k < HPL; ++k) {
    const uint32_t v = vl + k * kFoldThreads;
    if (v >= v1) continue;
    const bool inB = v >= vb;
    PM_G uint64_t* const par = (inB ? PB.parity : PA.parity) + (uint64_t)(v - (inB ? vb : hA)) * E;
    PM_G uint32_t* dst = reinterpret_cast<PM_G uint32_t*>(par + w);
    if (slice < npk) {
      typedef uint32_t u32x4 __attribute__((ext_vector_type(4)));
#pragma unroll
      for (int t = 0; t < 8; t += 2) {
        PM_G u32x4* const d = reinterpret_cast<PM_G u32x4*>(dst + 8 * (j ^ (t >> 2)) + 2 * (t & 3));
        const u32x4 x = {acc[k][t] << 16, acc[k][t] & 0xffff0000u, acc[k][t + 1] << 16, acc[k][t + 1] & 0xffff0000u};
        if (PM_PREP_NT) __builtin_nontemporal_store(x, d);
        else *d = x;
      }
    } else {
#pragma unroll
      for (int t = 0; t < 8; ++t) {
        PM_G uint32_t* const d = dst + 4 * (j ^ (t >> 2)) + (t & 3);
        if (PM_PREP_NT) __builtin_nontemporal_store(acc[k][t], d);
        else *d = acc[k][t];
      }
    }
    if (w == 0)
      for (uint32_t t = E & ~3u; t < E; ++t) par[t] = 0;
  }
}

__host__ __device__ inline FoldImageSrc fold_image_src(uint64_t x, uint32_t nbuf, uint32_t CS, uint32_t npk) {
  const uint32_t lg = CS == 512 ? 2 : 1;
  const uint32_t it = (uint32_t)(x % (kRotBufBytes / 16));
  const uint64_t blk = x / (kRotBufBytes / 16);
  const uint32_t b = (uint32_t)(blk % nbuf), s = (uint32_t)(blk / nbuf);
  FoldImageSrc o;
  o.row = (uint64_t)((b << lg) + ((it >> 1) & ((1u << lg) - 1))) * CS + (it >> (lg + 1));
  o.packed = s < npk;
  o.word = o.packed ? 16 * s + 8 * (it & 1) : 8 * (s + npk) + 4 * (it & 1);
  return o;
}
__global__ void __launch_bounds__(kBlock) k_fold_image(uint4* __restrict__ img, const uint64_t* __restrict__ rows,
                                                      uint64_t N, uint32_t nbuf, uint32_t E, uint64_t nitems,
                                                      uint32_t CS, uint32_t npk) {
  for (uint64_t x = (uint64_t)blockIdx.x * kBlock + threadIdx.x; x < nitems; x += (uint64_t)gridDim.x * kBlock) {
    const FoldImageSrc src = fold_image_src(x, nbuf, CS, npk);
    uint4 v = make_uint4(0, 0, 0, 0);
    if (src.row < N) {
      const uint4* const p = reinterpret_cast<const uint4*>(reinterpret_cast<const uint32_t*>(rows + src.row * E) + src.word);
      v = p[0];
      if (src.packed) {
        const uint4 u = p[1];
        v = make_uint4((v.x >> 16) | (v.y & 0xffff0000u), (v.z >> 16) | (v.w & 0xffff0000u),
                       (u.x >> 16) | (u.y & 0xffff0000u), (u.z >> 16) | (u.w & 0xffff0000u));
      }
    }
    img[x] = v;
  }
}
__global__ void __launch_bounds__(kBlock) k_coord_low_or(const uint64_t* __restrict__ rows, uint64_t nrows, uint32_t E,
                                                        uint32_t dim, uint32_t* __restrict__ out) {
  const uint32_t per = dim / 4;
  const uint64_t nitems = nrows * per;
  uint32_t acc = 0;
  for (uint64_t x = (uint64_t)blockIdx.x * kBlock + threadIdx.x; x < nitems; x += (uint64_t)gridDim.x * kBlock) {
    const uint64_t r = x / per;
    const uint4 v = reinterpret_cast<const uint4*>(rows + r * E)[x - r * per];
    acc |= v.x | v.y | v.z | v.w;
  }
  if (acc & 0xffffu) atomicOr(out, 1u);
}

constexpr uint32_t kReplRows = 32, kReplIt = (kReplRows * 1024 / 16 + kBlock - 1) / kBlock;
template <int W>
__global__ void __launch_bounds__(kBlock) k_prep_repl(const PmPart* __restrict__ parts,
                                                      const uint64_t* __restrict__ db, uint32_t E) {
  typedef uint64_t vec __attribute__((ext_vector_type(W)));
  __shared__ uint32_t rrow[kReplRows];
  const PmPart& P = parts[blockIdx.y];
  const uint32_t nslot = P.SS * P.Qpc;
  const uint32_t s0 = blockIdx.x * kReplRows;
  if (s0 >= nslot) return;
  const uint32_t ns = min(kReplRows, nslot - s0);
  if (threadIdx.x < ns) {
    const uint32_t slot = s0 + threadIdx.x, c = slot / P.Qpc;
    const uint64_t off = hash4(P.seed, DOM_REPL, P.idx, P.epoch, slot) & (P.CS - 1);
    const uint64_t r = (uint64_t)c * P.CS + off;
    P.ridx[slot] = (uint32_t)r;
    rrow[threadIdx.x] = r < P.N ? (uint32_t)r : ~0u;
  }
  __syncthreads();
  const uint32_t nseg = E / W, tot = ns * nseg;
  const uint64_t* const src = db + P.row0 * E;
  uint64_t* const dst = P.rval + (uint64_t)s0 * E;
  for (uint32_t x0 = 0; x0 < tot; x0 += kReplIt * kBlock) {
    vec v[kReplIt];
    uint32_t at[kReplIt];
#pragma unroll
    for (uint32_t u = 0; u < kReplIt; ++u) {
      const uint32_t x = x0 + u * kBlock + threadIdx.x;
      at[u] = ~0u;
      v[u] = vec{};
      if (x < tot) {
        const uint32_t i = x / nseg, sg = x - i * nseg, r = rrow[i];
        at[u] = i * E + sg * W;
        if (r != ~0u) v[u] = *reinterpret_cast<const vec*>(src + (uint64_t)r * E + sg * W);
      }
    }
#pragma unroll
    for (uint32_t u = 0; u < kReplIt; ++u)
      if (at[u] != ~0u) *reinterpret_cast<vec*>(dst + at[u]) = v[u];
  }
}

__global__ void __launch_bounds__(kBlock) k_prep_init(const PmPart* __restrict__ parts) {
  const PmPart& P = parts[blockIdx.y];
  const uint32_t i = blockIdx.x * kBlock + threadIdx.x;
  if (i < P.H) P.tag[i] = i;
  if (i < P.PH) P.pp[i] = kDefaultProgramPoint;
  if (i < P.SS) P.hist[i] = 0;
  if (i < P.SS * P.Qpc) P.ridx[i] = kDefaultProgramPoint;
  if (i == 0) *P.fqn = 0;
}

template <int W>
__global__ void __launch_bounds__(kBlock) k_server_answer(const PmPart* __restrict__ parts,
                                                          const uint32_t* __restrict__ qoffs,
                                                          uint32_t maxSS,
                                                          const uint64_t* __restrict__ db, uint32_t E,
                                                          uint64_t* __restrict__ ans) {
  __shared__ uint64_t red[kBlock * 2];
  const uint32_t s = blockIdx.x;
  const PmPart& P = parts[0];
  const uint32_t EX = E & ~3u, NSEG = EX / W;
  const uint32_t* qo = qoffs + (uint64_t)s * maxSS;
  const uint64_t* base = db + P.row0 * E;
  uint64_t* out = ans + (uint64_t)s * E;
  for (uint32_t seg0 = 0; seg0 < NSEG; seg0 += kBlock) {
    const uint32_t nseg = min(NSEG - seg0, (uint32_t)kBlock);
    const uint32_t nsl = kBlock / nseg;
    const uint32_t sl = threadIdx.x / nseg, seg = seg0 + threadIdx.x % nseg;
    uint64_t a0 = 0, a1 = 0;
// ... 149 lines not shown
    out[i] = prf64(A, srk, tags[i], xs[i]);
}

__global__ void __launch_bounds__(kBlock) k_gather_rows(const uint64_t* const* __restrict__ src, uint32_t E,
                                                         uint64_t* __restrict__ out) {
  const uint64_t i = blockIdx.x;
  const uint64_t* r = src[i];
  uint64_t* o = out + i * (E + 1);
  for (uint32_t w = threadIdx.x; w < E; w += kBlock) o[w] = r ? r[w] : 0;
  if (threadIdx.x == 0) o[E] = r ? 1 : 0;
}

}

namespace pmk {
static inline unsigned cdiv(uint64_t a, uint64_t b) { return (unsigned)((a + b - 1) / b); }

void prep_init(hipStream_t st, const PmPart* d, int np, uint32_t maxH, uint32_t maxRepl, uint32_t,
               bool) {
  const uint32_t n = maxH > maxRepl ? maxH : maxRepl;
  hipLaunchKernelGGL(k_prep_init, dim3(cdiv(n, kBlock), np), dim3(kBlock), 0, st, d);
}
void prep_offsets_tt(hipStream_t st, const PmPart* d, int np, uint32_t maxH, uint32_t maxSS) {
  hipLaunchKernelGGL(k_prep_offsets, dim3(cdiv(maxH, kOffsBlock), cdiv(maxSS, kOffsChunksPerBlock * kOffsTiles), np),
                     dim3(kOffsBlock), 0, st, d);
}
void prep_offsets_bs(hipStream_t st, const PmPart* d, int np, uint32_t maxH, uint32_t maxSS) {
  hipLaunchKernelGGL(k_prep_offsets_bs, dim3(cdiv((uint64_t)cdiv(maxH, 32) * cdiv(maxSS, 8), kBsThreads), np),
                     dim3(kBsThreads), 0, st, d);
}
static std::atomic<int> g_aes_bs{-1};
void set_aes_bs(int v) { g_aes_bs.store(v < 0 ? -1 : (v ? 1 : 0)); }
bool prep_offsets_bitsliced() {
  static const bool env = [] { const char* e = getenv("PM_AES_BS"); return e && e[0] == '1'; }();
  const int v = g_aes_bs.load();
  return v < 0 ? env : v == 1;
}
void prep_offsets(hipStream_t st, const PmPart* d, int np, uint32_t maxH, uint32_t maxSS) {
  if (prep_offsets_bitsliced()) prep_offsets_bs(st, d, np, maxH, maxSS);
  else prep_offsets_tt(st, d, np, maxH, maxSS);
}
static std::atomic<int> g_fold_rot{-1};
void set_fold_rot(int v) { g_fold_rot.store(v < 0 ? -1 : (v ? 1 : 0)); }
static bool fold_rot_shape(uint32_t minCS, uint32_t maxCS, uint32_t E) {
  return minCS == maxCS && (maxCS == 512 || maxCS == 1024) && E % 2 == 0 && E >= 4;
}
bool fold_image_ok(uint32_t minCS, uint32_t maxCS, uint32_t E) {
  static const bool env = [] { const char* e = getenv("PM_FOLD_ROT"); return !e || e[0] != '0'; }();
  const int v = g_fold_rot.load();
  return (v < 0 ? env : v == 1) && fold_rot_shape(minCS, maxCS, E);
}
static uint32_t fold_blk_sw(uint32_t maxCS) {
  auto fits = [&](uint32_t sw) {
    return 2ull * (maxCS + 1) * sw * 8 <= 150u * 1024 &&
           (uint64_t)maxCS * (sw / 2) <= (uint64_t)kFoldMaxItems * kFoldThreads;
  };
  uint32_t sw = 8;
  while (sw > 2 && !fits(sw)) sw /= 2;
  return fits(sw) ? sw : 0;
}
int fold_form(uint32_t minCS, uint32_t maxCS, uint32_t E, bool have_img, uint32_t npk) {
  if ((E & ~3u) == 0) return FOLD_GATHER;
  if (have_img && fold_rot_shape(minCS, maxCS, E))
    return maxCS == 512 ? (npk ? FOLD_ROT512P : FOLD_ROT512) : FOLD_ROT1024;
  if (minCS == maxCS && (maxCS == 512 || maxCS == 1024 || maxCS == 2048) && E % 2 == 0) return FOLD_PIPE;
  if (E % 2 || !fold_blk_sw(maxCS)) return FOLD_GATHER;
  return FOLD_BLK;
}
bool fold_needs_tab(uint32_t minCS, uint32_t maxCS, uint32_t E, bool have_img) {
  const int form = fold_form(minCS, maxCS, E, have_img);
  return form == FOLD_PIPE || form == FOLD_BLK;
}
static std::atomic<int> g_fold_pack{-1};
void set_fold_pack(int v) { g_fold_pack.store(v < 0 ? -1 : (v ? 1 : 0)); }
uint32_t fold_pack_slices(uint32_t minCS, uint32_t maxCS, uint32_t E, uint32_t dim) {
  static const bool env = [] { const char* e = getenv("PM_FOLD_PACK"); return !e || e[0] != '0'; }();
  const int v = g_fold_pack.load();
  if (!(v < 0 ? env : v == 1) || fold_form(minCS, maxCS, E, true) != FOLD_ROT512) return 0;
  return fold_pack_shape(E, dim);
}
uint32_t fold_pack_shape(uint32_t E, uint32_t dim) {
  return dim && dim % 16 == 0 && dim / 8 <= E / 4 ? dim / 16 : 0;
}
bool coord_low_zero(hipStream_t st, const uint64_t* rows, uint64_t nrows, uint32_t E, uint32_t dim, uint32_t* flag) {
  if (hipMemsetAsync(flag, 0, 4, st) != hipSuccess) return false;
  unsigned grid = cdiv(nrows * (dim / 4), kBlock);
  if (grid > 256 * 32) grid = 256 * 32;
  if (grid) hipLaunchKernelGGL(k_coord_low_or, dim3(grid), dim3(kBlock), 0, st, rows, nrows, E, dim, flag);
  uint32_t h = 1;
  if (hipMemcpyAsync(&h, flag, 4, hipMemcpyDeviceToHost, st) != hipSuccess || hipStreamSynchronize(st) != hipSuccess)
    return false;
  return h == 0;
}
uint64_t fold_image_words(uint32_t SS, uint32_t E, uint32_t CS, uint32_t npk) {
  return (uint64_t)(E / 4 - npk) * (SS / rot_nch(CS)) * (kRotBufBytes / 8);
}
void fold_image(hipStream_t st, uint64_t* img, const uint64_t* rows, uint64_t N, uint32_t SS, uint32_t E, uint32_t CS,
                uint32_t npk) {
  const uint64_t nitems = fold_image_words(SS, E, CS, npk) / 2;
  unsigned grid = cdiv(nitems, kBlock);
  if (grid > 256 * 32) grid = 256 * 32;
  hipLaunchKernelGGL(k_fold_image, dim3(grid), dim3(kBlock), 0, st, (uint4*)img, rows, N, SS / rot_nch(CS), E, nitems,
                     CS, npk);
}
void fold_image_map(uint32_t CS, uint32_t SS, uint32_t npk, uint64_t x0, uint64_t n, uint64_t* row, uint32_t* word,
                    uint8_t* packed) {
  for (uint64_t i = 0; i < n; ++i) {
    const FoldImageSrc s = fold_image_src(x0 + i, SS / rot_nch(CS), CS, npk);
    row[i] = s.row; word[i] = s.word; packed[i] = s.packed;
  }
}
int prep_fold(hipStream_t st, const PmPart* d, int np, uint32_t maxH, const uint64_t* db, uint32_t E,
              uint32_t minCS, uint32_t maxCS, const uint64_t* zero16, uint32_t clients, bool have_img,
               uint32_t minH, uint32_t npk) {
  const int form = fold_form(minCS, maxCS, E, have_img, npk);
  const uint32_t EX = E & ~3u;
  if (EX == 0) {
    hipLaunchKernelGGL(k_prep_fold<2>, dim3(cdiv((uint64_t)maxH * E, kBlock), np), dim3(kBlock), 0,
                       st, d, db, E);
    return form;
  }
  const uint32_t ng = cdiv(maxH, (uint64_t)kFoldThreads * kFoldHPT);
  const uint32_t ngb = cdiv(maxH, (uint64_t)kFoldThreads * kFoldHPTBlk);
  auto launch = [&](uint32_t sw, uint32_t w0, uint32_t nsl) {
    const size_t lds = 2ull * (maxCS + 1) * sw * 8;
    const dim3 grid(ngb, nsl, np), blk(kFoldThreads);
    if (sw == 8) hipLaunchKernelGGL(k_prep_fold_blk<8>, grid, blk, lds, st, d, db, zero16, E, w0);
    else if (sw == 4) hipLaunchKernelGGL(k_prep_fold_blk<4>, grid, blk, lds, st, d, db, zero16, E, w0);
    else hipLaunchKernelGGL(k_prep_fold_blk<2>, grid, blk, lds, st, d, db, zero16, E, w0);
  };
  if (form == FOLD_ROT512 || form == FOLD_ROT512P || form == FOLD_ROT1024 || form == FOLD_PIPE) {
    const uint32_t psw = maxCS == 2048 ? 2 : 4, nsl = EX / psw - (form == FOLD_ROT512P ? npk : 0);
    const uint32_t K = clients && np % clients == 0 ? clients : 1, npg = (np / K) * ng;
    const uint32_t lw = 16 / psw, per_pg = K * cdiv(nsl, lw) * lw;
#ifndef PM_FOLD_NB512
#define PM_FOLD_NB512 4
#endif
#ifndef PM_FOLD_D512
#define PM_FOLD_D512 1
#endif
    if (form != FOLD_PIPE) {
      const uint64_t HB = (uint64_t)kFoldThreads * rot_hpl(maxCS);
      const uint32_t ngc = minH >= HB ? 0u : (uint32_t)cdiv(maxH, HB);
      const uint32_t nvg = ngc ? K * ngc : (uint32_t)cdiv((uint64_t)K * maxH, HB), npv = (np / K) * nvg;
      const uint32_t grid = 8 * cdiv((uint64_t)cdiv(npv, PM_ROT_GB) * cdiv(nsl, PM_ROT_SB), 8) * PM_ROT_GB * PM_ROT_SB;
      if (form != FOLD_ROT1024)
        hipLaunchKernelGGL(k_prep_fold_rot<512>, dim3(grid), dim3(kFoldThreads), 0, st, d, E, nvg, nsl, npv,
                           form == FOLD_ROT512P ? npk : 0u, K, ngc);
      else
        hipLaunchKernelGGL(k_prep_fold_rot<1024>, dim3(grid), dim3(kFoldThreads), 0, st, d, E, nvg, nsl, npv, 0u, K, ngc);
      return form;
    }
    const uint32_t nb = maxCS == 512 ? PM_FOLD_NB512 : 3;
    const size_t lds = (size_t)nb * ((maxCS + 1) * psw + kPipeTabWords) * 8;
    const dim3 grid(cdiv(npg, 8) * 8 * per_pg), blk(kFoldThreads);
    if (maxCS == 512)
      hipLaunchKernelGGL((k_prep_fold_pipe<4, 1, PM_FOLD_NB512, PM_FOLD_D512>), grid, blk, lds, st, d, db, zero16, E, ng, nsl,
                         npg, K);
    else if (maxCS == 1024)
      hipLaunchKernelGGL((k_prep_fold_pipe<4, 2, 3>), grid, blk, lds, st, d, db, zero16, E, ng, nsl, npg, K);
    else
      hipLaunchKernelGGL((k_prep_fold_pipe<2, 2, 3>), grid, blk, lds, st, d, db, zero16, E, ng, nsl, npg, K);
    return form;
  }
  if (form == FOLD_GATHER) {
    if (E % 2 == 0)
// ... 73 lines not shown
```

pacmann_amd/csrc/pm_query.hip:

```cpp
#include <hip/hip_ext.h>

#include "pm_aes.h"
#include "pm_internal.h"
#include <atomic>
#include <climits>
#include <cstdlib>
#include <cstring>

namespace pm {

constexpr int kAnsBlock = 512;
#ifndef PM_ANSWER_NTLOAD
#define PM_ANSWER_NTLOAD 0
#endif
#ifndef PM_STEP_KG
#define PM_STEP_KG 12
#endif
#ifndef PM_ANSWER_KG
#define PM_ANSWER_KG 6
#endif
constexpr uint32_t kNone = 0xffffffffu;

#ifdef PM_STAMPS
#define STAMP(i)                                                                 \
// ... 1792 lines not shown
  __syncthreads();
  if (tid == 0) {
    __builtin_amdgcn_fence(__ATOMIC_RELEASE, "agent");
    asm volatile("s_waitcnt vmcnt(0)" ::: "memory");
    L.s_last = (uint32_t)chain_add(S, 1);
    if (L.s_last) {
      __builtin_amdgcn_fence(__ATOMIC_ACQUIRE, "agent");
      asm volatile("s_waitcnt vmcnt(0)" ::: "memory");
    }
  }
  __syncthreads();
  if (!L.s_last) return;
  finish_step<GRAN>(S, row);
}

template <int W>
#ifndef PM_ANSWER_WGS
#define PM_ANSWER_WGS 8
#endif
__global__ void __launch_bounds__(kAnsBlock, PM_ANSWER_WGS) k_answer(PmStep S) {
  __shared__ AnswerLds<kAnsBlock> L;
  answer_role<W, false, kAnsBlock>(S, blockIdx.x, L);
}

constexpr uint32_t kSmallSS = 1024, kSmallE = 256;
template <int W, int NT>
__global__ void __launch_bounds__(NT, PM_ANSWER_WGS) k_answer_s(PmStep S) {
  __shared__ AnswerLds<NT, kSmallSS, kSmallE> L;
  answer_role<W, false, NT>(S, blockIdx.x, L);
}

constexpr int kAnsPNT = 128;
template <int NT>
struct AnswerPLds {
  __attribute__((aligned(16))) uint16_t qo[2][kSmallSS];
  uint64_t red[NT * 2];
  __attribute__((aligned(16))) RowBufT<kSmallE> row;
  uint32_t s_last;
};
struct AnsQ {
  uint32_t s, part, mode;
  PmRes r;
  uint64_t idx;
  uint64_t e_rv, e_bp, e_pp;
  uint32_t e_cur;
  float q0, q1;
};
template <int W, int NT>
__device__ __forceinline__ void ansp_decode_ops(const PmStep& S, AnsQ& a) {
  const PmPart& P = S.parts[a.part];
  const uint32_t tid = threadIdx.x, E = S.E;
  a.e_rv = a.e_bp = a.e_pp = 0;
  a.e_cur = kSkip;
  if (a.mode != A_FINAL) return;
  const PmRes& r = a.r;
  const uint64_t dslot = (uint64_t)r.chunk * P.Qpc + r.ing;
  if (PM_DEC_NT) {
    if (!(r.flags & 2u) && tid < P.SS)
      a.e_cur = __builtin_nontemporal_load(P.tabT + tabT_index(P.H, P.PH + r.chunk * P.Qpc + r.ing, tid));
    if (tid < E) {
      a.e_rv = __builtin_nontemporal_load(P.rval + dslot * E + tid);
      a.e_bp = __builtin_nontemporal_load(P.parity + ((uint64_t)P.PH + dslot) * E + tid);
      a.e_pp = __builtin_nontemporal_load(P.parity + (uint64_t)r.hit * E + tid);
    }
    return;
  }
  if (!(r.flags & 2u) && tid < P.SS) a.e_cur = P.tabT[tabT_index(P.H, P.PH + r.chunk * P.Qpc + r.ing, tid)];
  if (tid < E) {
    a.e_rv = P.rval[dslot * E + tid];
    a.e_bp = P.parity[((uint64_t)P.PH + dslot) * E + tid];
    a.e_pp = P.parity[(uint64_t)r.hit * E + tid];
  }
}
__device__ __forceinline__ void ansp_set(const PmStep& S, const AnsQ& a, uint4 qpv, uint16_t* qo) {
  const uint32_t tid = threadIdx.x;
  if (a.mode == A_FINAL || a.mode == A_CHAINED) {
    if (tid < S.qw / 8) *reinterpret_cast<uint4*>(qo + 8 * tid) = qpv;
  } else if (a.mode == A_DUMMY) {
    const PmPart& P = S.parts[a.part];
    const uint32_t mask = P.CS - 1;
    for (uint32_t i = tid; i < P.SS; i += blockDim.x) qo[i] = (uint16_t)(hash4(P.seed, DOM_DUMMY, P.idx, a.idx, i) & mask);
  }
}
template <int W, int NT, int KG>
struct AnsGather {
  typedef uint64_t u64x2 __attribute__((ext_vector_type(2)));
  uint32_t seg, sl, nsl;
  uint64_t a0 = 0, a1 = 0;
  u64x2 x[KG];
  __device__ __forceinline__ void init(uint32_t E) {
    const uint32_t NSEG = (E & ~3u) / W;
    nsl = NT / NSEG;
    sl = threadIdx.x / NSEG;
    seg = threadIdx.x % NSEG;
  }
  __device__ __forceinline__ void load(const PmStep& S, const PmPart& P, const uint16_t* qo, uint32_t b) {
    const uint32_t i0 = sl + b * KG * nsl;
    uint32_t rr[KG];
#pragma unroll
    for (int u = 0; u < KG; ++u) rr[u] = qo[min(i0 + u * nsl, P.SS - 1)];
#pragma unroll
    for (int u = 0; u < KG; ++u) {
      const uint32_t i = i0 + u * nsl;
      rr[u] = (sl < nsl && i < P.SS) ? i * P.CS + rr[u] : ~0u;
    }
    const PM_G uint64_t* base = S.db + P.row0 * S.E;
#pragma unroll
    for (int u = 0; u < KG; ++u) {
      x[u] = u64x2{0, 0};
      if (rr[u] < P.N) {
        const PM_G uint64_t* q = base + (uint64_t)rr[u] * S.E + (uint64_t)seg * W;
#if PM_ANSWER_NTLOAD
        if (W == 2) x[u] = __builtin_nontemporal_load(reinterpret_cast<const PM_G u64x2*>(q));
        else x[u].x = __builtin_nontemporal_load(q);
#else
        if (W == 2) x[u] = *reinterpret_cast<const PM_G u64x2*>(q);
        else x[u].x = *q;
#endif
      }
    }
  }
  __device__ __forceinline__ void fold() {
#pragma unroll
    for (int u = 0; u < KG; ++u) { a0 ^= x[u].x; a1 ^= x[u].y; }
  }
  __device__ __forceinline__ uint32_t batches(const PmPart& P) const { return (P.SS + KG * nsl - 1) / (KG * nsl); }
  template <class LDS>
  __device__ __forceinline__ void reduce(LDS& L, uint32_t E) {
    const uint32_t tid = threadIdx.x, NSEG = (E & ~3u) / W;
    L.red[tid * 2] = a0;
    L.red[tid * 2 + 1] = a1;
    __syncthreads();
    if (tid < NSEG) {
      uint64_t x0 = 0, x1 = 0;
      for (uint32_t k = 0; k < nsl; ++k) {
        x0 ^= L.red[(k * NSEG + tid) * 2];
        x1 ^= L.red[(k * NSEG + tid) * 2 + 1];
      }
      L.row.w[tid * W] = x0;
      if (W == 2) L.row.w[tid * W + 1] = x1;
    }
    __syncthreads();
  }
};
template <int W, int NT, class LDS>
__device__ __forceinline__ void ansp_epilogue(const PmStep& S, const AnsQ& a, LDS& L) {
  const PmPart& P = S.parts[a.part];
  const PmRes& r = a.r;
  const uint32_t tid = threadIdx.x, E = S.E, EX = E & ~3u, s = a.s, mode = a.mode;
  auto& row = L.row;
  const uint64_t dslot = (uint64_t)r.chunk * P.Qpc + r.ing;
  uint64_t* pp = P.parity + (uint64_t)r.hit * E;
  if (mode == A_FINAL) {
    if (!(r.flags & 2u)) {
      if (tid < P.SS) {
        PM_G uint16_t* dst = P.cur + cur_index(P.PH, P.curk, tid, r.hit);
        if (PM_REFRESH_NT) __builtin_nontemporal_store((uint16_t)a.e_cur, dst);
        else *dst = (uint16_t)a.e_cur;
      }
      if (P.SS > NT) refresh_cur(P, r, tid + NT, NT);
    }
    const uint64_t* rv = P.rval + dslot * E;
    const uint64_t* bp = P.parity + ((uint64_t)P.PH + dslot) * E;
    for (uint32_t w = tid; w < E; w += NT) {
      const uint64_t rvw = w < NT ? a.e_rv : rv[w], bpw = w < NT ? a.e_bp : bp[w], ppw = w < NT ? a.e_pp : pp[w];
      uint64_t v = 0;
      if (w < EX) v = row.w[w] ^ rvw ^ ppw;
      const uint64_t nw = w < EX ? bpw ^ v : bpw;
      if (PM_EPI_NT) __builtin_nontemporal_store(nw, pp + w);
      else pp[w] = nw;
      row.w[w] = v;
    }
  } else if (mode == A_CHAINED) {
    for (uint32_t w = tid; w < E; w += NT) S.ans[(uint64_t)s * E + w] = w < EX ? row.w[w] : 0;
  } else if (mode == A_CACHED) {
    const uint64_t* ar = P.arena + (uint64_t)r.slot * E;
    for (uint32_t w = tid; w < E; w += NT) row.w[w] = ar[w];
  }
  const float* const qq = P.qv ? P.qv : S.q;
  const bool q_lds = qq && S.dim <= 2 * NT;
  float* const qf = reinterpret_cast<float*>(L.red);
  if (q_lds) {
    if (tid < S.dim) qf[tid] = a.q0;
    if (tid + NT < S.dim) qf[tid + NT] = a.q1;
  }
  __syncthreads();
  if (mode != A_CHAINED) {
    const bool has_row = (mode == A_FINAL || mode == A_CACHED);
    PM_G uint64_t* const orow = S.rows_h + (uint64_t)s * E;
    for (uint32_t w = (S.rows_partial ? S.pf_w0 : 0) + tid; w < (S.rows_partial ? S.pf_w1 : E); w += NT)
      row_store(orow + w, has_row ? row.w[w] : 0);
    if (mode == A_FINAL) {
      uint64_t* ar = P.arena + (uint64_t)r.slot * E;
      for (uint32_t w = tid; w < E; w += NT) {
        if (PM_EPI_NT) __builtin_nontemporal_store(row.w[w], ar + w);
        else ar[w] = row.w[w];
      }
    }
    float d = 0.0f;
    if (has_row && qq && tid < 8) d = l2_lds(row.f, q_lds ? qf : qq, S.dim);
    uint64_t cs = 0;
    if (tid < 64) cs = row_csum(S, row, has_row);
    publish_hdr(S, s, r.status, r.slot, d, cs);
  }
  if (r.status == ST_OK && (r.flags & 3u)) {
    asm volatile("s_waitcnt vmcnt(0)" ::: "memory");
    __syncthreads();
    if (tid == 0) {
      __builtin_amdgcn_fence(__ATOMIC_RELEASE, "agent");
      asm volatile("s_waitcnt vmcnt(0)" ::: "memory");
      L.s_last = (uint32_t)chain_add(S, 1);
      if (L.s_last) {
        __builtin_amdgcn_fence(__ATOMIC_ACQUIRE, "agent");
        asm volatile("s_waitcnt vmcnt(0)" ::: "memory");
      }
    }
    __syncthreads();
    if (L.s_last) finish_step<false>(S, row);
  }
  __syncthreads();
}
template <int W, int NT>
__device__ __forceinline__ void ansp_record(const PmStep& S, uint32_t s, AnsQ& a, uint4& qpv) {
  const uint32_t tid = threadIdx.x;
  a.s = s;
  const PmSub sub = step_sub(S, s);
  a.part = sub.part;
  a.idx = sub.idx;
  a.r = S.res[s];
  qpv = make_uint4(0, 0, 0, 0);
  if (tid < S.qw / 8) qpv = *reinterpret_cast<const PM_G uint4*>(S.qset + (uint64_t)s * S.qw + 8 * tid);
  const PmPart& P = S.parts[a.part];
  const float* const qq = P.qv ? P.qv : S.q;
  a.q0 = a.q1 = 0.0f;
  if (qq && S.dim <= 2 * NT) {
    if (tid < S.dim) a.q0 = qq[tid];
    if (tid + NT < S.dim) a.q1 = qq[tid + NT];
  }
}
__device__ __forceinline__ bool ansp_gathers(const AnsQ& a) {
  return a.mode == A_FINAL || a.mode == A_CHAINED || a.mode == A_DUMMY;
}
template <int W, int NT, int KG, int C>
__device__ __forceinline__ bool ansp_turn(const PmStep& S, AnswerPLds<NT>& L, AnsQ (&q)[2], uint4 (&qpv)[2],
                                          AnsGather<W, NT, KG> (&g)[2], uint32_t k, bool first) {
  constexpr int N = C ^ 1;
  const uint32_t ns = S.nsub, G = gridDim.x;
  const bool hasN = blockIdx.x + (k + 1) * G < ns;
  if (ansp_gathers(q[C])) {
    const PmPart& P = S.parts[q[C].part];
    const uint32_t nb = g[C].batches(P);
    uint32_t b = 0;
    if (!first) { g[C].fold(); b = 1; }
    for (; b < nb; ++b) {
      g[C].load(S, P, L.qo[C], b);
      g[C].fold();
    }
  }
  const bool gathN = hasN && ansp_gathers(q[N]);
  if (gathN) {
    g[N].a0 = g[N].a1 = 0;
    g[N].load(S, S.parts[q[N].part], L.qo[N], 0);
  }
  if (ansp_gathers(q[C])) g[C].reduce(L, S.E);
  ansp_epilogue<W, NT>(S, q[C], L);
  if (!hasN) return false;
  if (blockIdx.x + (k + 2) * G < ns) {
    ansp_record<W, NT>(S, blockIdx.x + (k + 2) * G, q[C], qpv[C]);
    q[C].mode = answer_mode(q[C].r);
    ansp_set(S, q[C], qpv[C], L.qo[C]);
    __syncthreads();
  }
  ansp_decode_ops<W, NT>(S, q[N]);
  return true;
}
#ifndef PM_ANSWER_PK_MAX
#define PM_ANSWER_PK_MAX 2
#endif
#ifndef PM_ANSWER_P_WAVES
#define PM_ANSWER_P_WAVES 6
#endif
template <int W, int NT, int KG>
__device__ __forceinline__ void answer_p_body(const PmStep& S, AnswerPLds<NT>& L) {
  AnsQ q[2];
  uint4 qpv[2];
  const uint32_t ns = S.nsub, G = gridDim.x;
  const bool has1 = blockIdx.x + G < ns;
  ansp_record<W, NT>(S, blockIdx.x, q[0], qpv[0]);
  ansp_record<W, NT>(S, has1 ? blockIdx.x + G : blockIdx.x, q[1], qpv[1]);
  q[0].mode = answer_mode(q[0].r);
  q[1].mode = answer_mode(q[1].r);
  ansp_decode_ops<W, NT>(S, q[0]);
  ansp_set(S, q[0], qpv[0], L.qo[0]);
  if (has1) ansp_set(S, q[1], qpv[1], L.qo[1]);
  __syncthreads();
  AnsGather<W, NT, KG> g[2];
  g[0].init(S.E);
  g[1].init(S.E);
  static_assert(PM_ANSWER_PK_MAX >= 2 && PM_ANSWER_PK_MAX <= 4, "k_answer_p turns");
  if (!ansp_turn<W, NT, KG, 0>(S, L, q, qpv, g, 0, true)) return;
  if (!ansp_turn<W, NT, KG, 1>(S, L, q, qpv, g, 1, false)) return;
  if (PM_ANSWER_PK_MAX > 2 && !ansp_turn<W, NT, KG, 0>(S, L, q, qpv, g, 2, false)) return;
  if (PM_ANSWER_PK_MAX > 3) ansp_turn<W, NT, KG, 1>(S, L, q, qpv, g, 3, false);
}
template <int W, int NT>
__global__ void __launch_bounds__(NT, PM_ANSWER_P_WAVES) k_answer_p(PmStep S) {
  __shared__ AnswerPLds<NT> L;
  answer_p_body<W, NT, PM_ANSWER_KG>(S, L);
}
constexpr int kAnsP5KG = 7;
template <int W, int NT>
__global__ void __launch_bounds__(NT, 5) __attribute__((amdgpu_num_vgpr(88))) k_answer_p5(PmStep S) {
  __shared__ AnswerPLds<NT> L;
  answer_p_body<W, NT, kAnsP5KG>(S, L);
}

constexpr int kGatherBlock = 256;
constexpr uint32_t kGatherMaxRange = 4096;
#ifndef PM_GATHER_NT
#define PM_GATHER_NT 1
#endif
#ifndef PM_GATHER_KG
#define PM_GATHER_KG 8
#endif
#ifndef PM_GATHER_WAVES
#define PM_GATHER_WAVES 8
#endif
template <int W>
__global__ void __launch_bounds__(kGatherBlock, PM_GATHER_WAVES) k_gather(PmStep S) {
  __shared__ uint64_t red[kGatherBlock * 2];
  __shared__ uint32_t rows_l[kGatherMaxRange];
  const uint32_t j = blockIdx.x, s = blockIdx.y, tid = threadIdx.x;
  const PmRes r = S.res[s];
  const uint32_t mode = answer_mode(r);
  if (mode != A_FINAL && mode != A_CHAINED && mode != A_DUMMY) return;
  const PmSub sub = step_sub(S, s);
  const PmPart& P = S.parts[sub.part];
  const uint32_t E = S.E, EX = E & ~3u, NSEG = EX / W, mask = P.CS - 1, lg = P.log2CS;
  const uint32_t per = (P.SS + S.nsplit - 1) / S.nsplit, c0 = min(P.SS, j * per), c1 = min(P.SS, c0 + per);
  const bool real = mode != A_DUMMY;
  const uint32_t pchunk = real && r.pp != kDefaultProgramPoint ? (r.pp >> lg) : kNone;
  const uint32_t rchunk = real ? r.chunk : kNone;
  const uint32_t rep = real && rchunk - c0 < c1 - c0 ? (P.ridx[r.chunk * P.Qpc + r.ing] & mask) : 0;
  for (uint32_t i = c0 + tid; i < c1; i += kGatherBlock) {
    uint32_t o;
    if (real) {
      o = P.tabT[tabT_index(P.H, r.tag, i)];
      if (i == pchunk) o = r.pp & mask;
      if (i == rchunk) o = rep;
    } else {
      o = (uint32_t)(hash4(P.seed, DOM_DUMMY, P.idx, sub.idx, i) & mask);
    }
    const uint64_t row = (uint64_t)i * P.CS + o;
    rows_l[i - c0] = row < P.N ? (uint32_t)row : ~0u;
  }
  __syncthreads();

  const PM_G uint64_t* base = S.db + P.row0 * E;
  PM_G uint64_t* out = S.part_x + ((uint64_t)s * S.nsplit + j) * EX;
  typedef uint64_t u64x2 __attribute__((ext_vector_type(2)));
  const uint32_t nr = c1 - c0;
  for (uint32_t seg0 = 0; seg0 < NSEG; seg0 += kGatherBlock) {
    const uint32_t nseg = min(NSEG - seg0, (uint32_t)kGatherBlock);
    const uint32_t nsl = kGatherBlock / nseg;
    const uint32_t sl = tid / nseg, seg = seg0 + tid % nseg;
    uint64_t a0 = 0, a1 = 0;
    if (sl < nsl) {
      constexpr int kG = PM_GATHER_KG;
      for (uint32_t i0 = sl; i0 < nr; i0 += kG * nsl) {
        uint32_t rr[kG];
#pragma unroll
        for (int u = 0; u < kG; ++u) rr[u] = rows_l[min(i0 + u * nsl, nr - 1)];
#pragma unroll
        for (int u = 0; u < kG; ++u)
          if (i0 + u * nsl >= nr) rr[u] = ~0u;
        u64x2 x[kG];
#pragma unroll
        for (int u = 0; u < kG; ++u) {
          x[u] = u64x2{0, 0};
          if (rr[u] != ~0u) {
            const PM_G uint64_t* q = base + (uint64_t)rr[u] * E + (uint64_t)seg * W;
            if (W == 2) x[u] = PM_GATHER_NT ? __builtin_nontemporal_load(reinterpret_cast<const PM_G u64x2*>(q))
                                         : *reinterpret_cast<const PM_G u64x2*>(q);
            else x[u].x = PM_GATHER_NT ? __builtin_nontemporal_load(q) : *q;
          }
        }
#pragma unroll
        for (int u = 0; u < kG; ++u) { a0 ^= x[u].x; a1 ^= x[u].y; }
      }
    }
    red[tid * 2] = a0;
    red[tid * 2 + 1] = a1;
    __syncthreads();
    if (tid < nseg) {
      uint64_t x0 = 0, x1 = 0;
      for (uint32_t k = 0; k < nsl; ++k) {
        x0 ^= red[(k * nseg + tid) * 2];
// ... 122 lines not shown
  p.np_live = s.np_live;
  if (!s.unfused && s.args_valid && s.granules && mpp <= kSpecSubs && s.maxPH <= kLdsPH &&
      2 * s.nsub + s.np <= kStepMaxWg) {
    p.cblk = 1;
    p.no_guess = s.no_guess ? 1u : 0u;
    if (O.step_help > 0 && (s.E & ~3u) <= kHelpWords && 2 * s.nsub + s.np < kStepResidentWg)
      p.nhelp = std::min(std::min(kStepHelpMax, (uint32_t)O.step_help), (kStepResidentWg - 2 * s.nsub - s.np) / s.nsub);
    p.at[STAGE_FUSED] = {FORM_STEP, 2 * s.nsub + s.np + p.nhelp * s.nsub, 1, kStepBlock};
    return p;
  }
  p.cblk = step_match_blocks(s.maxPH);
  const bool lds = mpp > kSpecSubs && s.maxPH <= kLdsPH && mpp * words <= kLdsBitWords;
  p.nsplit = 1;
  if (!s.no_split && s.maxSS >= 256 && s.nsub) {
    uint32_t n = O.gather_split > 0 ? (uint32_t)O.gather_split : std::min(cdiv(s.maxSS, 48), cdiv(4096, s.nsub));
    n = std::max(1u, std::min(n, 64u));
    if (n > 1) p.nsplit = std::max(n, cdiv(s.maxSS, kGatherMaxRange));
  }
  const bool mr = O.match_resolve && !lds && !s.args_valid && s.desc_shared && s.np >= 128 && s.nsub >= 4 * s.np &&
                  words <= 256;
  if (mr) {
    const bool small = O.match_resolve == 1 && mpp <= kSpecSubs && s.ph8 && s.maxPH <= 16u * kResolveBlockG;
    static_assert(16u * kResolveBlockG <= 8u * 256 * 4, "k_match_resolve_s<4, 256> holds every small shape");
    if (small) {
      p.np_live = 0;
      p.at[STAGE_MR] = {s.maxPH <= 8u * 256 * 2 ? FORM_MR_S2 : FORM_MR_S4, s.np, 1, 256};
      p.qset = s.maxSS <= kSmallSS && p.nsplit <= 1;
      if (p.qset) p.qw = (s.maxSS + 7) & ~7u;
    } else {
      p.at[STAGE_MR] = {FORM_MR_GENERAL, s.np, 1, kResolveBlockG};
    }
  } else {
    const int mode = O.match_part;
    const bool part = mode == 1 || (mode == -1 && s.np >= 128 && s.nsub >= 4 * s.np);
    const bool part8 = s.ph8 && O.match_part8 && mpp <= kPart8Subs &&
                       (part || (mode == -1 && s.np >= 64 && s.nsub >= 2 * s.np));
    if (part8) p.at[STAGE_MATCH] = {MATCH_PART8, cdiv(p.cblk, PM_MATCHPART8_NW), s.np, 64 * PM_MATCHPART8_NW};
    else if (part) p.at[STAGE_MATCH] = {MATCH_PART, p.cblk, s.np, kBlock};
    else p.at[STAGE_MATCH] = {MATCH_SUB, p.cblk, s.nsub, kBlock};
    if (lds) p.at[STAGE_RESOLVE] = {FORM_RESOLVE_LDS, s.np, 1, kBlock};
    else p.at[STAGE_RESOLVE] = {FORM_RESOLVE_G, s.np, 1, kResolveBlockG};
  }
  if (p.nsplit > 1) p.at[STAGE_GATHER] = {FORM_GATHER, p.nsplit, s.nsub, kGatherBlock};
  static_assert(2u * kAnsPNT >= kSmallE, "k_answer_p's gather slices must cover a kSmallE row");
  const bool search_sized = p.nsplit <= 1 && s.maxSS <= kSmallSS && s.E <= kSmallE;
  if (O.answer_pair && p.qset && search_sized && s.E % 2 == 0 && (s.E & ~3u) <= 2u * kAnsPNT && s.nsub >= 2 * 256) {
    const bool p5 = O.answer_waves == 5 || (O.answer_waves == 0 && s.E <= 80);
    p.at[STAGE_ANSWER] = {p5 ? FORM_ANSWER_P5 : FORM_ANSWER_P, cdiv(s.nsub, PM_ANSWER_PK_MAX), 1, kAnsPNT};
  } else if (O.answer_nt && search_sized) {
    p.at[STAGE_ANSWER] = {FORM_ANSWER_S, s.nsub, 1, O.answer_nt == 128 ? 128u : O.answer_nt == 512 ? 512u : 256u};
  } else {
    p.at[STAGE_ANSWER] = {FORM_ANSWER_G, s.nsub, 1, kAnsBlock};
  }
  return p;
}

#define PM_LAUNCH(kern)                                                                            \
  do {                                                                                             \
    if (ev.a) hipExtLaunchKernelGGL(kern, grid, blk, 0, st, ev.a, ev.b, 0, S);                      \
    else hipLaunchKernelGGL(kern, grid, blk, 0, st, S);                                            \
  } while (0)
#define PM_LAUNCH_W(kern, ...)                                                                     \
  do {                                                                                             \
    if (S.E % 2 == 0) PM_LAUNCH((kern<2, ##__VA_ARGS__>));                                         \
    else PM_LAUNCH((kern<1, ##__VA_ARGS__>));                                                      \
  } while (0)
void step_launch(hipStream_t st, const PmStep& S, const StepPlan& plan, int stage, PmEvents ev) {
  const StepLaunch& L = plan.at[stage];
  const dim3 grid(L.gx, L.gy), blk(L.block);
  if (stage == STAGE_MATCH) {
    if (L.form == MATCH_PART8) PM_LAUNCH(k_match_part8<PM_MATCHPART8_NW>);
    else if (L.form == MATCH_PART) PM_LAUNCH(k_match_part<kMatchHints / kBlock>);
    else PM_LAUNCH(k_match);
    return;
  }
  switch (L.form) {
    case FORM_STEP: PM_LAUNCH_W(k_step); break;
    case FORM_RESOLVE_LDS: PM_LAUNCH(k_resolve<true>); break;
    case FORM_RESOLVE_G: PM_LAUNCH(k_resolve<false>); break;
    case FORM_MR_S2: PM_LAUNCH((k_match_resolve_s<2, 256>)); break;
    case FORM_MR_S4: PM_LAUNCH((k_match_resolve_s<4, 256>)); break;
    case FORM_MR_GENERAL: PM_LAUNCH(k_match_resolve<kMatchHints / kBlock>); break;
    case FORM_GATHER: PM_LAUNCH_W(k_gather); break;
    case FORM_ANSWER_P5: PM_LAUNCH((k_answer_p5<2, kAnsPNT>)); break;
    case FORM_ANSWER_P: PM_LAUNCH((k_answer_p<2, kAnsPNT>)); break;
    case FORM_ANSWER_S:
      if (L.block == 128) PM_LAUNCH_W(k_answer_s, 128);
      else if (L.block == 512) PM_LAUNCH_W(k_answer_s, 512);
      else PM_LAUNCH_W(k_answer_s, 256);
      break;
    case FORM_ANSWER_G: PM_LAUNCH_W(k_answer); break;
  }
}
uint32_t step_max_sub_per_part() { return kMaxSubPerPart; }
uint32_t step_max_ss() { return kMaxSSLds; }
uint32_t step_max_e() { return kMaxELds; }
}
```

Measured before the change: 24910.

## Gather PIR answers from a packed 16-bit-coordinate database image

At setup, when the low 16 bits of each coordinate word are zero, builds a second device copy of the database in which every pair of coordinates is squeezed into one 32-bit word. It adds packed variants of the answer_p and answer_p5 kernels that gather and XOR-reduce rows from this narrower image, then unpack the result in LDS. This cuts the bytes read per row in the bandwidth-bound answer scan. The cost is extra HBM for the image (only built if it fits in a quarter of free memory), a one-time packing pass, and more kernel variants with different gather depths.

```diff
diff --git a/pacmann_amd/csrc/pm_ctx.cpp b/pacmann_amd/csrc/pm_ctx.cpp
--- a/pacmann_amd/csrc/pm_ctx.cpp
+++ b/pacmann_amd/csrc/pm_ctx.cpp
@@ -131,6 +131,11 @@
     pmk::set_fold_pack(value);
     return 0;
   }
+  if (!strcmp(name, "answer_pack")) {
+    if (value < -1 || value > 1) return fail(PM_EINVAL, "answer_pack takes 1, 0 or -1");
+    pmk::set_answer_pack(value);
+    return 0;
+  }
   if (pmk::set_option(name, value)) return fail(PM_EINVAL, std::string("unknown option ") + name);
   return 0;
 }
diff --git a/pacmann_amd/csrc/pm_devloop.cpp b/pacmann_amd/csrc/pm_devloop.cpp
--- a/pacmann_amd/csrc/pm_devloop.cpp
+++ b/pacmann_amd/csrc/pm_devloop.cpp
@@ -211,7 +211,7 @@
   S.subs_h = S.subs;
   S.sb_h = S.sb;
   S.done = G.done.as<uint32_t>();
-  S.db = e0->db->as<uint64_t>();
+  e0->step_db(S);
   S.q = nullptr;
   step_out(S, T.out.p, T.nsub);
   S.E = G.E; S.dim = G.dim; S.nsub = T.nsub; S.np = T.S * G.Pl;
diff --git a/pacmann_amd/csrc/pm_engine.cpp b/pacmann_amd/csrc/pm_engine.cpp
--- a/pacmann_amd/csrc/pm_engine.cpp
+++ b/pacmann_amd/csrc/pm_engine.cpp
@@ -129,16 +129,19 @@
     HIPCHK(hipStreamSynchronize(ctx->stream));
   }
   uint64_t off_img = 0;
-  if (!g->owned_list.empty() && pmk::fold_image_ok(g->minCS, g->maxCS, (uint32_t)g->E)) {
-    if (server) {
-      g->img_npk = server->img_npk;
-    } else if (const uint32_t npk = pmk::fold_pack_slices(g->minCS, g->maxCS, (uint32_t)g->E, coord_words)) {
-      DevBuf flag;
-      CHK(flag.reserve(64));
-      if (pmk::coord_low_zero(ctx->stream, g->db->as<uint64_t>(), off_db, (uint32_t)g->E, coord_words, flag.as<uint32_t>()))
-        g->img_npk = npk;
-      HIPCHK(hipGetLastError());
-    }
+  const bool fold_img = !g->owned_list.empty() && pmk::fold_image_ok(g->minCS, g->maxCS, (uint32_t)g->E);
+  const uint32_t want_npk = !server && fold_img ? pmk::fold_pack_slices(g->minCS, g->maxCS, (uint32_t)g->E, coord_words) : 0;
+  const uint32_t want_apk = !server && !g->owned_list.empty() ? pmk::answer_pack_segs((uint32_t)g->E, coord_words) : 0;
+  bool low_zero = false;
+  if (want_npk || want_apk) {
+    DevBuf flag;
+    CHK(flag.reserve(64));
+    low_zero = pmk::coord_low_zero(ctx->stream, g->db->as<uint64_t>(), off_db, (uint32_t)g->E, coord_words, flag.as<uint32_t>());
+    HIPCHK(hipGetLastError());
+  }
+  if (fold_img) {
+    if (server) g->img_npk = server->img_npk;
+    else if (low_zero) g->img_npk = want_npk;
     for (uint32_t i : g->owned_list) {
       PmPart& d = g->parts[i].d;
       d.img = (const uint64_t*)(uintptr_t)off_img;
@@ -166,6 +169,19 @@
       }
       HIPCHK(hipGetLastError());
       HIPCHK(hipStreamSynchronize(ctx->stream));
+    }
+  }
+  if (server) {
+    g->apk = server->apk; g->apk_nseg = server->apk_nseg; g->apk_cseg = server->apk_cseg;
+  } else if (want_apk && low_zero) {
+    const uint64_t bytes = off_db * want_apk * 16;
+    size_t free_b = 0, total_b = 0;
+    if (hipMemGetInfo(&free_b, &total_b) != hipSuccess || bytes <= free_b / 4) {
+      CHK(g->apk->reserve(bytes));
+      pmk::answer_pack_image(ctx->stream, g->apk->as<uint64_t>(), g->db->as<uint64_t>(), off_db, (uint32_t)g->E, coord_words);
+      HIPCHK(hipGetLastError());
+      HIPCHK(hipStreamSynchronize(ctx->stream));
+      g->apk_nseg = want_apk; g->apk_cseg = coord_words / 8;
     }
   }
   CHK(g->tag.reserve(off_tag * 4));
@@ -623,6 +639,7 @@
     if (form < 0) return;
     c->timed_ext(name, bytes, [&](pmk::PmEvents ev) { pmk::step_launch(st, S, plan, stage, ev); }, 2);
     c->host_add(pm_ctx::step_counter(stage, form), stage == pmk::STAGE_FUSED ? plan.nhelp : 0.0);
+    if (pmk::step_answer_packed(S, plan, stage)) c->host_add(HT_ANSWER_PACKED, 0.0);
   };
 #ifdef PM_STEP_STAMPS
   LaunchStamps ss;
@@ -695,7 +712,7 @@
   HIPCHK(hipMemsetAsync(B.stamps.p, 0, g->P * 64 * 8, st));
   S.stamps = B.stamps.as<uint64_t>();
 #endif
-  S.db = g->db->as<uint64_t>();
+  g->step_db(S);
   S.q = q_dev;
   step_out(S, B.out_h.p, nsub);
   S.E = (uint32_t)E; S.dim = q_dev ? dim : 0; S.nsub = nsub; S.np = (uint32_t)g->P;
diff --git a/pacmann_amd/csrc/pm_engine.h b/pacmann_amd/csrc/pm_engine.h
--- a/pacmann_amd/csrc/pm_engine.h
+++ b/pacmann_amd/csrc/pm_engine.h
@@ -180,6 +180,13 @@
   std::shared_ptr<DevBuf> db = std::make_shared<DevBuf>();
   std::shared_ptr<DevBuf> img = std::make_shared<DevBuf>();
   uint32_t img_npk = 0;
+  std::shared_ptr<DevBuf> apk = std::make_shared<DevBuf>();
+  uint32_t apk_nseg = 0, apk_cseg = 0;
+  void step_db(PmStep& S) const {
+    S.db = db->as<uint64_t>();
+    S.dbp = apk_nseg ? apk->as<uint64_t>() : nullptr;
+    S.pk_nseg = apk_nseg; S.pk_cseg = apk_cseg;
+  }
   DevBuf zero16, parts_d, owned_d, tag, pp, parity, ridx, rval, hist, fqn, arena, tab, tabT, cur, done, gran;
   HostBuf parts_stage;
   hipEvent_t stage_ev = nullptr;
diff --git a/pacmann_amd/csrc/pm_group.cpp b/pacmann_amd/csrc/pm_group.cpp
--- a/pacmann_amd/csrc/pm_group.cpp
+++ b/pacmann_amd/csrc/pm_group.cpp
@@ -206,7 +206,7 @@
   }
   S.done = G.done.as<uint32_t>();
   Engine* e0 = G.es[0];
-  S.db = e0->db->as<uint64_t>();
+  e0->step_db(S);
   S.q = nullptr;
   if (G.comb) {
     CHK(G.out_d.reserve(step_out_bytes(nsub, G.E)));
diff --git a/pacmann_amd/csrc/pm_host.h b/pacmann_amd/csrc/pm_host.h
--- a/pacmann_amd/csrc/pm_host.h
+++ b/pacmann_amd/csrc/pm_host.h
@@ -80,8 +80,8 @@
   template <class T> T* as() const { return (T*)p; }
 };
 
-enum HostTimer : int { HT_STEP_LAUNCH, HT_STEP_WAIT, HT_STEP_POST, HT_BATCH_QUERY, HT_GVI_PARSE, HT_SEARCH_KNN, HT_KNN_INIT, HT_KNN_BATCH, HT_KNN_UPDATE, HT_KNN_FINAL, HT_WAIT_FIRST, HT_WAIT_ALL, HT_ROWS_SEEN, HT_ROWS_TORN, HT_WAIT_DONE, HT_COMBINE, HT_COMBINE_TURN, HT_PATH_MATCH, HT_PATH_MATCH_PART, HT_PATH_MATCH_PART8, HT_PREP_SETS, HT_REC_VERIFIED, HT_REC_BAD, HT_REC_DROPPED, HT_REC_FAILED, HT_REC_PEER, HT_REC_UNEXPLAINED, HT_FOLD_ROT512, HT_FOLD_ROT1024, HT_FOLD_OTHER, HT_FOLD_PIPE, HT_FOLD_BLK, HT_FOLD_GATHER, HT_FOLD_ROT512P, HT_DEV_STEPS, HT_DEV_QUERIES, HT_KNN_BATCH_FALLBACK, HT_PATH_STEP, HT_PATH_RESOLVE_LDS, HT_PATH_RESOLVE_G, HT_PATH_MR_S2, HT_PATH_MR_S4, HT_PATH_MR_GENERAL, HT_PATH_GATHER, HT_PATH_ANSWER_P5, HT_PATH_ANSWER_P, HT_PATH_ANSWER_S, HT_PATH_ANSWER_G, HT_COUNT };
-static const char* const kHostTimerName[HT_COUNT] = {"host_step_launch", "host_step_wait", "host_step_post", "host_batch_query", "host_gvi_parse", "host_search_knn", "host_knn_init", "host_knn_batch", "host_knn_update", "host_knn_final", "host_wait_first_token", "host_wait_all_tokens", "host_rows_seen", "host_rows_torn", "host_wait_done", "host_combine", "host_combine_turn", "host_path_match", "host_path_match_part", "host_path_match_part8", "host_prep_sets", "host_records_verified", "host_records_bad", "host_records_dropped", "host_records_failed", "host_records_peer", "host_records_unexplained", "host_fold_rot512", "host_fold_rot1024", "host_fold_other", "host_fold_pipe", "host_fold_blk", "host_fold_gather", "host_fold_rot512p", "host_dev_steps", "host_dev_queries", "host_knn_batch_fallback", "host_path_step", "host_path_resolve_lds", "host_path_resolve_g", "host_path_mr_s2", "host_path_mr_s4", "host_path_mr_general", "host_path_gather", "host_path_answer_p5", "host_path_answer_p", "host_path_answer_s", "host_path_answer_g"};
+enum HostTimer : int { HT_STEP_LAUNCH, HT_STEP_WAIT, HT_STEP_POST, HT_BATCH_QUERY, HT_GVI_PARSE, HT_SEARCH_KNN, HT_KNN_INIT, HT_KNN_BATCH, HT_KNN_UPDATE, HT_KNN_FINAL, HT_WAIT_FIRST, HT_WAIT_ALL, HT_ROWS_SEEN, HT_ROWS_TORN, HT_WAIT_DONE, HT_COMBINE, HT_COMBINE_TURN, HT_PATH_MATCH, HT_PATH_MATCH_PART, HT_PATH_MATCH_PART8, HT_PREP_SETS, HT_REC_VERIFIED, HT_REC_BAD, HT_REC_DROPPED, HT_REC_FAILED, HT_REC_PEER, HT_REC_UNEXPLAINED, HT_FOLD_ROT512, HT_FOLD_ROT1024, HT_FOLD_OTHER, HT_FOLD_PIPE, HT_FOLD_BLK, HT_FOLD_GATHER, HT_FOLD_ROT512P, HT_DEV_STEPS, HT_DEV_QUERIES, HT_KNN_BATCH_FALLBACK, HT_PATH_STEP, HT_PATH_RESOLVE_LDS, HT_PATH_RESOLVE_G, HT_PATH_MR_S2, HT_PATH_MR_S4, HT_PATH_MR_GENERAL, HT_PATH_GATHER, HT_PATH_ANSWER_P5, HT_PATH_ANSWER_P, HT_PATH_ANSWER_S, HT_PATH_ANSWER_G, HT_ANSWER_PACKED, HT_COUNT };
+static const char* const kHostTimerName[HT_COUNT] = {"host_step_launch", "host_step_wait", "host_step_post", "host_batch_query", "host_gvi_parse", "host_search_knn", "host_knn_init", "host_knn_batch", "host_knn_update", "host_knn_final", "host_wait_first_token", "host_wait_all_tokens", "host_rows_seen", "host_rows_torn", "host_wait_done", "host_combine", "host_combine_turn", "host_path_match", "host_path_match_part", "host_path_match_part8", "host_prep_sets", "host_records_verified", "host_records_bad", "host_records_dropped", "host_records_failed", "host_records_peer", "host_records_unexplained", "host_fold_rot512", "host_fold_rot1024", "host_fold_other", "host_fold_pipe", "host_fold_blk", "host_fold_gather", "host_fold_rot512p", "host_dev_steps", "host_dev_queries", "host_knn_batch_fallback", "host_path_step", "host_path_resolve_lds", "host_path_resolve_g", "host_path_mr_s2", "host_path_mr_s4", "host_path_mr_general", "host_path_gather", "host_path_answer_p5", "host_path_answer_p", "host_path_answer_s", "host_path_answer_g", "host_answer_packed"};
 static_assert(HT_PATH_ANSWER_G - HT_PATH_STEP + 1 == pmk::FORM_COUNT, "one counter per step form, in the order of pmk::FORM_*");
 
 struct TimedLaunch { std::string name; hipEvent_t a, b; double bytes; };
diff --git a/pacmann_amd/csrc/pm_internal.h b/pacmann_amd/csrc/pm_internal.h
--- a/pacmann_amd/csrc/pm_internal.h
+++ b/pacmann_amd/csrc/pm_internal.h
@@ -133,6 +133,8 @@
   PM_G uint64_t* ans;
   PM_G uint32_t* done;
   const PM_G uint64_t* db;
+  const PM_G uint64_t* dbp;
+  uint32_t pk_nseg, pk_cseg;
   const PM_G float* q;
   PM_G PmOutHdr* hdr_h;
   PM_G uint64_t* rows_h;
@@ -236,6 +238,10 @@
 uint32_t fold_pack_shape(uint32_t E, uint32_t dim);
 uint32_t fold_pack_slices(uint32_t minCS, uint32_t maxCS, uint32_t E, uint32_t dim);
 bool coord_low_zero(hipStream_t st, const uint64_t* rows, uint64_t nrows, uint32_t E, uint32_t dim, uint32_t* flag);
+void set_answer_pack(int v);
+uint32_t answer_pack_shape(uint32_t E, uint32_t dim);
+uint32_t answer_pack_segs(uint32_t E, uint32_t dim);
+void answer_pack_image(hipStream_t st, uint64_t* img, const uint64_t* rows, uint64_t nrows, uint32_t E, uint32_t dim);
 void fold_image_map(uint32_t CS, uint32_t SS, uint32_t npk, uint64_t x0, uint64_t n, uint64_t* row, uint32_t* word,
                     uint8_t* packed);
 struct PmEvents { hipEvent_t a = nullptr, b = nullptr; };
@@ -271,6 +277,10 @@
 };
 StepPlan step_plan(const StepShape& s, const StepOpts& O);
 void step_launch(hipStream_t st, const PmStep& S, const StepPlan& plan, int stage, PmEvents ev = {});
+inline bool step_answer_packed(const PmStep& S, const StepPlan& plan, int stage) {
+  const int form = plan.at[stage].form;
+  return stage == STAGE_ANSWER && (form == FORM_ANSWER_P5 || form == FORM_ANSWER_P) && S.dbp != nullptr;
+}
 uint32_t step_max_sub_per_part();
 uint32_t step_max_ss();
 uint32_t step_max_e();
diff --git a/pacmann_amd/csrc/pm_kernels.hip b/pacmann_amd/csrc/pm_kernels.hip
--- a/pacmann_amd/csrc/pm_kernels.hip
+++ b/pacmann_amd/csrc/pm_kernels.hip
@@ -630,6 +630,24 @@
     img[x] = v;
   }
 }
+__global__ void __launch_bounds__(kBlock) k_answer_pack_image(uint4* __restrict__ img, const uint64_t* __restrict__ rows,
+                                                             uint64_t nitems, uint32_t E, uint32_t nseg, uint32_t cseg) {
+  for (uint64_t x = (uint64_t)blockIdx.x * kBlock + threadIdx.x; x < nitems; x += (uint64_t)gridDim.x * kBlock) {
+    const uint64_t r = x / nseg;
+    const uint32_t s = (uint32_t)(x - r * nseg);
+    const uint32_t* const row = reinterpret_cast<const uint32_t*>(rows + r * E);
+    uint4 v;
+    if (s < cseg) {
+      const uint4* const p = reinterpret_cast<const uint4*>(row + 8 * s);
+      const uint4 a = p[0], u = p[1];
+      v = make_uint4((a.x >> 16) | (a.y & 0xffff0000u), (a.z >> 16) | (a.w & 0xffff0000u),
+                     (u.x >> 16) | (u.y & 0xffff0000u), (u.z >> 16) | (u.w & 0xffff0000u));
+    } else {
+      v = *reinterpret_cast<const uint4*>(row + 8 * cseg + 4 * (s - cseg));
+    }
+    img[x] = v;
+  }
+}
 __global__ void __launch_bounds__(kBlock) k_coord_low_or(const uint64_t* __restrict__ rows, uint64_t nrows, uint32_t E,
                                                         uint32_t dim, uint32_t* __restrict__ out) {
   const uint32_t per = dim / 4;
@@ -945,6 +963,25 @@
 uint32_t fold_pack_shape(uint32_t E, uint32_t dim) {
   return dim && dim % 16 == 0 && dim / 8 <= E / 4 ? dim / 16 : 0;
 }
+static std::atomic<int> g_answer_pack{-1};
+void set_answer_pack(int v) { g_answer_pack.store(v < 0 ? -1 : (v ? 1 : 0)); }
+uint32_t answer_pack_shape(uint32_t E, uint32_t dim) {
+  if (!dim || E % 4 || E > 256 || dim % 8 || dim >= 2 * E) return 0;
+  const uint32_t stride = 2 * dim + 4 * (2 * E - dim);
+  return stride % 16 ? 0 : stride / 16;
+}
+uint32_t answer_pack_segs(uint32_t E, uint32_t dim) {
+  static const bool env = [] { const char* e = getenv("PM_ANSWER_PACK"); return !e || e[0] != '0'; }();
+  const int v = g_answer_pack.load();
+  return (v < 0 ? env : v == 1) ? answer_pack_shape(E, dim) : 0;
+}
+void answer_pack_image(hipStream_t st, uint64_t* img, const uint64_t* rows, uint64_t nrows, uint32_t E, uint32_t dim) {
+  const uint32_t nseg = answer_pack_shape(E, dim);
+  const uint64_t nitems = nrows * nseg;
+  unsigned grid = cdiv(nitems, kBlock);
+  if (grid > 256 * 32) grid = 256 * 32;
+  if (grid) hipLaunchKernelGGL(k_answer_pack_image, dim3(grid), dim3(kBlock), 0, st, (uint4*)img, rows, nitems, E, nseg, dim / 8);
+}
 bool coord_low_zero(hipStream_t st, const uint64_t* rows, uint64_t nrows, uint32_t E, uint32_t dim, uint32_t* flag) {
   if (hipMemsetAsync(flag, 0, 4, st) != hipSuccess) return false;
   unsigned grid = cdiv(nrows * (dim / 4), kBlock);
diff --git a/pacmann_amd/csrc/pm_query.hip b/pacmann_amd/csrc/pm_query.hip
--- a/pacmann_amd/csrc/pm_query.hip
+++ b/pacmann_amd/csrc/pm_query.hip
@@ -1898,14 +1898,16 @@
     for (uint32_t i = tid; i < P.SS; i += blockDim.x) qo[i] = (uint16_t)(hash4(P.seed, DOM_DUMMY, P.idx, a.idx, i) & mask);
   }
 }
-template <int W, int NT, int KG>
+template <int W, int NT, int KG, bool PK>
 struct AnsGather {
   typedef uint64_t u64x2 __attribute__((ext_vector_type(2)));
+  static_assert(!PK || W == 2, "packed rows are gathered in 16-B segments");
   uint32_t seg, sl, nsl;
   uint64_t a0 = 0, a1 = 0;
   u64x2 x[KG];
-  __device__ __forceinline__ void init(uint32_t E) {
-    const uint32_t NSEG = (E & ~3u) / W;
+  __device__ __forceinline__ uint32_t nseg(const PmStep& S) const { return PK ? S.pk_nseg : (S.E & ~3u) / W; }
+  __device__ __forceinline__ void init(const PmStep& S) {
+    const uint32_t NSEG = nseg(S);
     nsl = NT / NSEG;
     sl = threadIdx.x / NSEG;
     seg = threadIdx.x % NSEG;
@@ -1920,12 +1922,13 @@
       const uint32_t i = i0 + u * nsl;
       rr[u] = (sl < nsl && i < P.SS) ? i * P.CS + rr[u] : ~0u;
     }
-    const PM_G uint64_t* base = S.db + P.row0 * S.E;
+    const uint32_t stride = PK ? S.pk_nseg * 2 : S.E;
+    const PM_G uint64_t* base = (PK ? S.dbp : S.db) + P.row0 * stride;
 #pragma unroll
     for (int u = 0; u < KG; ++u) {
       x[u] = u64x2{0, 0};
       if (rr[u] < P.N) {
-        const PM_G uint64_t* q = base + (uint64_t)rr[u] * S.E + (uint64_t)seg * W;
+        const PM_G uint64_t* q = base + (uint64_t)rr[u] * stride + (uint64_t)seg * W;
 #if PM_ANSWER_NTLOAD
         if (W == 2) x[u] = __builtin_nontemporal_load(reinterpret_cast<const PM_G u64x2*>(q));
         else x[u].x = __builtin_nontemporal_load(q);
@@ -1942,8 +1945,8 @@
   }
   __device__ __forceinline__ uint32_t batches(const PmPart& P) const { return (P.SS + KG * nsl - 1) / (KG * nsl); }
   template <class LDS>
-  __device__ __forceinline__ void reduce(LDS& L, uint32_t E) {
-    const uint32_t tid = threadIdx.x, NSEG = (E & ~3u) / W;
+  __device__ __forceinline__ void reduce(LDS& L, const PmStep& S) {
+    const uint32_t tid = threadIdx.x, NSEG = nseg(S);
     L.red[tid * 2] = a0;
     L.red[tid * 2 + 1] = a1;
     __syncthreads();
@@ -1953,8 +1956,16 @@
         x0 ^= L.red[(k * NSEG + tid) * 2];
         x1 ^= L.red[(k * NSEG + tid) * 2 + 1];
       }
-      L.row.w[tid * W] = x0;
-      if (W == 2) L.row.w[tid * W + 1] = x1;
+      if (PK && tid < S.pk_cseg) {
+        L.row.w[tid * 4] = ((x0 & 0xffffull) << 16) | ((x0 & 0xffff0000ull) << 32);
+        L.row.w[tid * 4 + 1] = ((x0 >> 16) & 0xffff0000ull) | (x0 & 0xffff000000000000ull);
+        L.row.w[tid * 4 + 2] = ((x1 & 0xffffull) << 16) | ((x1 & 0xffff0000ull) << 32);
+        L.row.w[tid * 4 + 3] = ((x1 >> 16) & 0xffff0000ull) | (x1 & 0xffff000000000000ull);
+      } else {
+        const uint32_t w = PK ? S.pk_cseg * 4 + (tid - S.pk_cseg) * 2 : tid * W;
+        L.row.w[w] = x0;
+        if (W == 2) L.row.w[w + 1] = x1;
+      }
     }
     __syncthreads();
   }
@@ -2057,9 +2068,9 @@
 __device__ __forceinline__ bool ansp_gathers(const AnsQ& a) {
   return a.mode == A_FINAL || a.mode == A_CHAINED || a.mode == A_DUMMY;
 }
-template <int W, int NT, int KG, int C>
+template <int W, int NT, int KG, bool PK, int C>
 __device__ __forceinline__ bool ansp_turn(const PmStep& S, AnswerPLds<NT>& L, AnsQ (&q)[2], uint4 (&qpv)[2],
-                                          AnsGather<W, NT, KG> (&g)[2], uint32_t k, bool first) {
+                                          AnsGather<W, NT, KG, PK> (&g)[2], uint32_t k, bool first) {
   constexpr int N = C ^ 1;
   const uint32_t ns = S.nsub, G = gridDim.x;
   const bool hasN = blockIdx.x + (k + 1) * G < ns;
@@ -2078,7 +2089,7 @@
     g[N].a0 = g[N].a1 = 0;
     g[N].load(S, S.parts[q[N].part], L.qo[N], 0);
   }
-  if (ansp_gathers(q[C])) g[C].reduce(L, S.E);
+  if (ansp_gathers(q[C])) g[C].reduce(L, S);
   ansp_epilogue<W, NT>(S, q[C], L);
   if (!hasN) return false;
   if (blockIdx.x + (k + 2) * G < ns) {
@@ -2096,7 +2107,7 @@
 #ifndef PM_ANSWER_P_WAVES
 #define PM_ANSWER_P_WAVES 6
 #endif
-template <int W, int NT, int KG>
+template <int W, int NT, int KG, bool PK = false>
 __device__ __forceinline__ void answer_p_body(const PmStep& S, AnswerPLds<NT>& L) {
   AnsQ q[2];
   uint4 qpv[2];
@@ -2110,14 +2121,14 @@
   ansp_set(S, q[0], qpv[0], L.qo[0]);
   if (has1) ansp_set(S, q[1], qpv[1], L.qo[1]);
   __syncthreads();
-  AnsGather<W, NT, KG> g[2];
-  g[0].init(S.E);
-  g[1].init(S.E);
+  AnsGather<W, NT, KG, PK> g[2];
+  g[0].init(S);
+  g[1].init(S);
   static_assert(PM_ANSWER_PK_MAX >= 2 && PM_ANSWER_PK_MAX <= 4, "k_answer_p turns");
-  if (!ansp_turn<W, NT, KG, 0>(S, L, q, qpv, g, 0, true)) return;
-  if (!ansp_turn<W, NT, KG, 1>(S, L, q, qpv, g, 1, false)) return;
-  if (PM_ANSWER_PK_MAX > 2 && !ansp_turn<W, NT, KG, 0>(S, L, q, qpv, g, 2, false)) return;
-  if (PM_ANSWER_PK_MAX > 3) ansp_turn<W, NT, KG, 1>(S, L, q, qpv, g, 3, false);
+  if (!ansp_turn<W, NT, KG, PK, 0>(S, L, q, qpv, g, 0, true)) return;
+  if (!ansp_turn<W, NT, KG, PK, 1>(S, L, q, qpv, g, 1, false)) return;
+  if (PM_ANSWER_PK_MAX > 2 && !ansp_turn<W, NT, KG, PK, 0>(S, L, q, qpv, g, 2, false)) return;
+  if (PM_ANSWER_PK_MAX > 3) ansp_turn<W, NT, KG, PK, 1>(S, L, q, qpv, g, 3, false);
 }
 template <int W, int NT>
 __global__ void __launch_bounds__(NT, PM_ANSWER_P_WAVES) k_answer_p(PmStep S) {
@@ -2129,6 +2140,22 @@
 __global__ void __launch_bounds__(NT, 5) __attribute__((amdgpu_num_vgpr(88))) k_answer_p5(PmStep S) {
   __shared__ AnswerPLds<NT> L;
   answer_p_body<W, NT, kAnsP5KG>(S, L);
+}
+#ifndef PM_ANSWER_PK5_KG
+#define PM_ANSWER_PK5_KG 9
+#endif
+#ifndef PM_ANSWER_PK_KG
+#define PM_ANSWER_PK_KG 6
+#endif
+template <int W, int NT>
+__global__ void __launch_bounds__(NT, PM_ANSWER_P_WAVES) k_answer_pk(PmStep S) {
+  __shared__ AnswerPLds<NT> L;
+  answer_p_body<W, NT, PM_ANSWER_PK_KG, true>(S, L);
+}
+template <int W, int NT>
+__global__ void __launch_bounds__(NT, 5) __attribute__((amdgpu_num_vgpr(88))) k_answer_p5k(PmStep S) {
+  __shared__ AnswerPLds<NT> L;
+  answer_p_body<W, NT, PM_ANSWER_PK5_KG, true>(S, L);
 }
 
 constexpr int kGatherBlock = 256;
@@ -2417,8 +2444,14 @@
     case FORM_MR_S4: PM_LAUNCH((k_match_resolve_s<4, 256>)); break;
     case FORM_MR_GENERAL: PM_LAUNCH(k_match_resolve<kMatchHints / kBlock>); break;
     case FORM_GATHER: PM_LAUNCH_W(k_gather); break;
-    case FORM_ANSWER_P5: PM_LAUNCH((k_answer_p5<2, kAnsPNT>)); break;
-    case FORM_ANSWER_P: PM_LAUNCH((k_answer_p<2, kAnsPNT>)); break;
+    case FORM_ANSWER_P5:
+      if (step_answer_packed(S, plan, stage)) PM_LAUNCH((k_answer_p5k<2, kAnsPNT>));
+      else PM_LAUNCH((k_answer_p5<2, kAnsPNT>));
+      break;
+    case FORM_ANSWER_P:
+      if (step_answer_packed(S, plan, stage)) PM_LAUNCH((k_answer_pk<2, kAnsPNT>));
+      else PM_LAUNCH((k_answer_p<2, kAnsPNT>));
+      break;
     case FORM_ANSWER_S:
       if (L.block == 128) PM_LAUNCH_W(k_answer_s, 128);
       else if (L.block == 512) PM_LAUNCH_W(k_answer_s, 512);
```

New measurement: 28820 (median of 6 runs). +15.7%, better.
